# Alexyskoutnev/Quadruped-Trajectory-Optimization-Stack

Measured on AMD Instinct MI355X. Metric: NLP solves/sec (100-knot SOLO12 trot gait, 5 s horizon, converged to 1e-4); CoM L-inf vs TOWR in `parity`, higher is better.
Workload: dtype f64

## Files before the change

include/qtos_planner.h:

```cpp
#ifndef QTOS_PLANNER_H
#define QTOS_PLANNER_H

#ifdef __cplusplus
extern "C" {
#endif

#define QTOS_NEE 4
#define QTOS_MAX_PHASES 32
#define QTOS_START_DOUBLES 24
#define QTOS_CSV_COLS 37

typedef struct QtosParams {
  int n_phases[QTOS_NEE];
  double phase_dur[QTOS_NEE][QTOS_MAX_PHASES];
  double dt_base, dt_dyn, dt_rom;
  int force_polys_per_stance;
  double mass, gravity, inertia_b[9];
  double nominal_stance[QTOS_NEE][3], max_dev[3];
  double mu, f_max, t_swing_avg;
  int honor_start_velocity;
  int terrain_mode;
  int max_iter;
  double tol, mu_init, mu_min, delta_x, eps_dual;
  double slack_push;
// ... 100 lines not shown
  double step_size;
  double tol;
  double z_offset;
  double cell, origin_x, origin_y;
  double t_stop, stop_dist;
  int base;
  int clamp_x, advance_clock, hold_done;
  int n_paths, max_pieces;
  int n_maps, rows, cols;
} QtosPathGoal;
int qtos_path_goal_device(QtosPlanner *p, int B, const QtosPathGoal *g, const double *d_knots, const double *d_coef,
                          const int *d_n_pieces, const double *d_robot_goal , const int *d_path_id ,
                          const double *d_height_yx , const int *d_map_id , double *d_clock ,
                          const double *d_offset , const double *d_start , double *d_goal_out,
                          int *d_done , void *stream);
int qtos_path_goal(QtosPlanner *p, int B, const QtosPathGoal *g, const double *knots, const double *coef, const int *n_pieces,
                   const double *robot_goal, const int *path_id, const double *height_yx, const int *map_id, double *clock,
                   const double *offset, const double *start, double *goal_out, int *done);

typedef struct QtosPathPlan {
  int rows, cols;
  double cell, origin_x, origin_y;
  double height_bound;
  double step_size;
  int max_cells;
  int max_open;
  int max_pieces;
  int n_maps;
  int set_done;
} QtosPathPlan;
int qtos_path_plan_device(QtosPlanner *p, int B, const QtosPathPlan *g, const double *d_bool_maps, const int *d_map_id ,
                          const double *d_start, const double *d_robot_goal, double *d_knots, double *d_coef, int *d_n_pieces,
                          int *d_cells , int *d_n_cells, int *d_status, int *d_done , void *stream);
int qtos_path_plan(QtosPlanner *p, int B, const QtosPathPlan *g, const double *bool_maps, const int *map_id, const double *start,
                   const double *robot_goal, double *knots, double *coef, int *n_pieces, int *cells, int *n_cells, int *status, int *done);

typedef struct QtosProbe {
  int rows, cols;
  int n_maps;
  double cell;
  int scale;
  int multi_map_shift;
  double origin_shift;
  double z_offset;
  double nominal_stance[QTOS_NEE][3];
} QtosProbe;
int qtos_probe_device(QtosPlanner *p, const QtosProbe *g, const double *d_map_yx, int capacity, int *d_offsets, int *d_slot, int *d_patch,
                      double *d_start , double *d_goal , int *d_map_id , void *stream);
int qtos_probe(QtosPlanner *p, const QtosProbe *g, const double *map_yx, int capacity, int *offsets, int *slot, int *patch, double *start,
               double *goal, int *map_id);
int qtos_probe_stamp_device(QtosPlanner *p, const QtosProbe *g, const int *d_offsets, const int *d_slot, const int *d_patch ,
                            const int *d_status, double *d_bool_maps, void *stream);
int qtos_probe_stamp(QtosPlanner *p, const QtosProbe *g, const int *offsets, const int *slot, const int *patch, const int *status,
                     double *bool_maps);

#define QTOS_ENV_MAX_LEVELS 64
#define QTOS_ENV_MAX_DRAWS (1 << 24)
#define QTOS_ENV_LDS_BYTES 3568
typedef struct QtosTerrainEnv {
  int n_maps;
  int n_base;
  int rows, cols;
  int n_shift;
  int n_height;
  int climb;
  double delta;
} QtosTerrainEnv;
int qtos_terrain_env_device(QtosPlanner *p, const QtosTerrainEnv *g, const double *d_base_yx, const int *d_base_id ,
                            const unsigned long long *d_seed, int *d_draws , double *d_map_yx,
                            double *d_height_xy , int *d_status, void *stream);
int qtos_terrain_env(QtosPlanner *p, const QtosTerrainEnv *g, const double *base_yx, const int *base_id, const unsigned long long *seed,
                     int *draws, double *map_yx, double *height_xy, int *status);

int qtos_write_csv(const char *path, const double *rows, int n_rows, int n_threads);

int qtos_plan_submit(QtosPlanner *p, int B, const double *d_start, const double *d_goal,
                     const int *d_map_id, const double *d_warm, double *d_nodes_out,
                     int *d_status_out, int *d_iters_out, double *d_viol_out, void *stream);
int qtos_plan_poll(QtosPlanner *p, int *done);
int qtos_plan_wait(QtosPlanner *p);
int qtos_set_speculation(QtosPlanner *p, int max_blind_iterations);
int qtos_set_pattern_speculation(QtosPlanner *p, int on);
int qtos_env(const QtosPlanner *p, char *buf, int n);

int qtos_last_timing(QtosPlanner *p, double *kkt_seconds, int *kkt_launches, double *total_seconds,
                     int *iterations);
int qtos_last_timing_detail(QtosPlanner *p, double *out, int n_out);
int qtos_set_kernel_events(QtosPlanner *p, int on);
int qtos_set_report(QtosPlanner *p, int on);

#define QTOS_HIST_COLS 10
enum {
  QTOS_H_INF_PR = 0,
  QTOS_H_THETA,
  QTOS_H_MU,
  QTOS_H_DNORM,
  QTOS_H_ALPHA_PR,
  QTOS_H_ALPHA_DU,
  QTOS_H_LS,
  QTOS_H_KIND,
  QTOS_H_COMPL,
  QTOS_H_INF_DU
};

typedef struct QtosReport {
  int status;
  int iterations;
  int n_rows;
  int n_con_evals;
  int n_jac_evals;
  int n_factorizations;
  int n_chord_solves;
  int pad;
  double constraint_violation;
  double dual_infeasibility;
  double complementarity;
  double nlp_error;
} QtosReport;
int qtos_plan_report(QtosPlanner *p, int b, QtosReport *out, double *rows, int max_rows);
int qtos_analyze_counts(const QtosParams *params, long long *counts, int n);

int qtos_last_timing_chord(QtosPlanner *p, double *chord_seconds, int *chord_launches);
int qtos_plan_totals(QtosPlanner *p, long long *converged, long long *iterations, int reset);

int qtos_debug_eval(QtosPlanner *p, int B, const double *start, const double *goal,
                    const int *map_id, const double *nodes, double *g_out, double *J_out);
int qtos_debug_newton(QtosPlanner *p, int B, const double *start, const double *goal,
                      const int *map_id, const double *nodes, const double *sig, const double *w,
                      double *dx_out);
int qtos_debug_chord(QtosPlanner *p, int B, double *dx_out);
int qtos_project_nodes(QtosPlanner *p, int B, const double *nodes, double *nodes_out);
int qtos_debug_stream_len(const QtosPlanner *p);
int qtos_debug_read_stream(QtosPlanner *p, int b, double *out);
int qtos_debug_read_rhs(QtosPlanner *p, int b, double *out);
int qtos_debug_residual(QtosPlanner *p, int B, int refine, double *dx_out, double *res_rel_out);
int qtos_debug_structure(const QtosPlanner *p, int *row_kind, int *var_free, int *order);
int qtos_debug_factor(QtosPlanner *p, int b, double *panel_out, int *piv_slot_out);
int qtos_debug_initial_guess(QtosPlanner *p, int B, const double *start, const double *goal,
                             const int *map_id, double *nodes_out);
int qtos_debug_trace(QtosPlanner *p, int b, double *trace_out);
int qtos_debug_duals(QtosPlanner *p, int B, double *s, double *zl, double *zu, double *y);
int qtos_build_flags(void);
int qtos_kkt_kernel(const QtosPlanner *p, char *buf, int n);
int qtos_analyze_kernel(const QtosParams *params, char *buf, int n);

typedef struct QtosSelftest {
  int order_rule, front, n_stages;
  int n_problems;
  int worst_stage;
  int passed;
  double residual;
  double residual_refined;
  double max_factor;
  double growth_limit;
  double tol_residual;
  double seconds;
} QtosSelftest;
int qtos_planner_selftest(QtosPlanner *p, unsigned long long seed, double tol_residual, QtosSelftest *out);
int qtos_selftest_inputs(const QtosParams *params, unsigned long long seed, int b, double *dx0, double *sig, double *w);
unsigned long long qtos_selftest_bits(unsigned long long seed, int problem, int array, unsigned long long index);
int qtos_selftest_problem(const QtosParams *params, double *start, double *goal);
int qtos_planner_create_checked(const QtosParams *params, int max_batch, int device, int rules_mask, double tol_residual,
                                QtosPlanner **out, QtosSelftest *tried, int max_tried, int *n_tried);
int qtos_analyze_candidates(const QtosParams *params, int rules_mask, int *rules, int *fronts, int *stages, int n);

#ifdef __cplusplus
// ... 4 lines not shown
```

quadruped-trajectory-optimization-stack_amd/capi.py:

```python
import ctypes as C
import os

import numpy as np

_HERE = os.path.dirname(os.path.abspath(__file__))
LIB_PATH = os.path.join(_HERE, "csrc", os.environ.get("QTOS_LIB", "libqtos_planner.so"))
NEE, MAX_PHASES, START_DOUBLES, CSV_COLS = 4, 32, 24, 37


class QtosParams(C.Structure):
    _fields_ = [
        ("n_phases", C.c_int * NEE),
        ("phase_dur", (C.c_double * MAX_PHASES) * NEE),
        ("dt_base", C.c_double), ("dt_dyn", C.c_double), ("dt_rom", C.c_double),
        ("force_polys_per_stance", C.c_int),
        ("mass", C.c_double), ("gravity", C.c_double), ("inertia_b", C.c_double * 9),
        ("nominal_stance", (C.c_double * 3) * NEE), ("max_dev", C.c_double * 3),
        ("mu", C.c_double), ("f_max", C.c_double), ("t_swing_avg", C.c_double),
        ("honor_start_velocity", C.c_int), ("terrain_mode", C.c_int),
        ("max_iter", C.c_int),
        ("tol", C.c_double), ("mu_init", C.c_double), ("mu_min", C.c_double),
        ("delta_x", C.c_double), ("eps_dual", C.c_double), ("slack_push", C.c_double), ("warm_slack_push", C.c_double),
        ("stall_iters", C.c_int), ("hold_from", C.c_int), ("hold_weight", C.c_double), ("hold_tol", C.c_double),
        ("chord_tol", C.c_double),
# ... 154 lines not shown
    return g


class QtosProbe(C.Structure):
    _fields_ = [
        ("rows", C.c_int), ("cols", C.c_int), ("n_maps", C.c_int), ("cell", C.c_double), ("scale", C.c_int), ("multi_map_shift", C.c_int),
        ("origin_shift", C.c_double), ("z_offset", C.c_double), ("nominal_stance", (C.c_double * 3) * NEE),
    ]

    def copy(self):
        return QtosProbe.from_buffer_copy(self)


def probe_params(map_yx=None, multi_map_shift=1, scale=1, origin_shift=1.0, cell=0.1, z_offset=0.24,
                 nominal_stance=((0.21, 0.19, 0.0), (0.21, -0.19, 0.0), (-0.21, 0.19, 0.0), (-0.21, -0.19, 0.0))):
    g = QtosProbe()
    g.cell, g.scale, g.multi_map_shift = float(cell), int(scale), int(multi_map_shift)
    g.origin_shift, g.z_offset = float(origin_shift), float(z_offset)
    for e in range(NEE):
        for k in range(3):
            g.nominal_stance[e][k] = float(nominal_stance[e][k])
    if map_yx is not None:
        is_shape = isinstance(map_yx, (tuple, list)) and len(map_yx) in (2, 3) and all(isinstance(v, (int, np.integer)) for v in map_yx)
        shape = tuple(int(v) for v in (map_yx if is_shape else np.shape(map_yx)))
        if len(shape) not in (2, 3):
            raise ValueError("map_yx is n_maps x rows x cols or rows x cols, or that shape")
        g.n_maps, g.rows, g.cols = (1,) + shape if len(shape) == 2 else shape
    return g


class QtosTerrainEnv(C.Structure):
    _fields_ = [
        ("n_maps", C.c_int), ("n_base", C.c_int), ("rows", C.c_int), ("cols", C.c_int), ("n_shift", C.c_int), ("n_height", C.c_int),
        ("climb", C.c_int), ("delta", C.c_double),
    ]

    def copy(self):
        return QtosTerrainEnv.from_buffer_copy(self)


ENV_MAX_LEVELS, ENV_MAX_DRAWS, ENV_LDS_BYTES = 64, 1 << 24, 3568


def terrain_env_params(base_yx=None, n_maps=None, n_shift=10, n_height=10, climb=False, delta=0.005):
    g = QtosTerrainEnv()
    g.n_shift, g.n_height, g.climb, g.delta = int(n_shift), int(n_height), int(bool(climb)), float(delta)
    if base_yx is not None:
        is_shape = isinstance(base_yx, (tuple, list)) and len(base_yx) in (2, 3) and all(isinstance(v, (int, np.integer)) for v in base_yx)
        shape = tuple(int(v) for v in (base_yx if is_shape else np.shape(base_yx)))
        if len(shape) not in (2, 3):
            raise ValueError("base_yx is n_base x rows x cols or rows x cols, or that shape")
        g.n_base, g.rows, g.cols = (1,) + shape if len(shape) == 2 else shape
        g.n_maps = g.n_base
    if n_maps is not None:
        g.n_maps = int(n_maps)
    return g


class SelftestError(RuntimeError):

    def __init__(self, attempts):
        self.attempts = attempts
        RuntimeError.__init__(self, "no elimination order passed the KKT self-test: " + "; ".join(a.describe() for a in attempts))


MAX_TRIED = 3

EXPORTS = [
    "qtos_planner_create", "qtos_planner_destroy", "qtos_planner_dims", "qtos_last_error",
    "qtos_set_heightfields", "qtos_plan_batch", "qtos_plan_batch_device", "qtos_sample_csv",
    "qtos_sample_csv_device", "qtos_last_timing", "qtos_debug_eval", "qtos_debug_newton",
    "qtos_debug_structure", "qtos_debug_trace", "qtos_debug_factor", "qtos_analyze", "qtos_analyze_sweep", "qtos_analyze_kron",
    "qtos_set_init_table", "qtos_debug_initial_guess", "qtos_shift_warm", "qtos_shift_warm_device",
    "qtos_last_timing_chord", "qtos_debug_chord", "qtos_plan_totals",
    "qtos_plan_submit", "qtos_plan_poll", "qtos_plan_wait", "qtos_set_speculation", "qtos_debug_residual", "qtos_project_nodes",
    "qtos_debug_stream_len", "qtos_debug_read_stream", "qtos_debug_read_rhs", "qtos_build_flags", "qtos_kkt_kernel",
    "qtos_last_timing_detail", "qtos_set_pattern_speculation", "qtos_env", "qtos_analyze_two_ended", "qtos_analyze_order", "qtos_set_kernel_events",
    "qtos_write_csv", "qtos_set_report", "qtos_plan_report", "qtos_analyze_counts", "qtos_debug_duals", "qtos_analyze_kernel",
    "qtos_planner_selftest", "qtos_planner_create_checked", "qtos_analyze_candidates", "qtos_selftest_inputs", "qtos_selftest_bits",
    "qtos_selftest_problem", "qtos_handover", "qtos_handover_device", "qtos_stitch", "qtos_stitch_device",
    "qtos_path_goal", "qtos_path_goal_device", "qtos_path_plan", "qtos_path_plan_device",
    "qtos_probe", "qtos_probe_device", "qtos_probe_stamp", "qtos_probe_stamp_device",
    "qtos_terrain_env", "qtos_terrain_env_device", "qtos_set_heightfields_device",
]

_lib = None


def load():
    global _lib
    if _lib is not None:
        return _lib
    if not os.path.exists(LIB_PATH):
        raise OSError("HIP planner library not built: %s (run __graft_entry__.build()); "
                      "this package has no CPU fallback" % LIB_PATH)
    try:
        import importlib.util
        spec = importlib.util.find_spec("torch")
        for loc in (spec.submodule_search_locations or []) if spec else []:
            hip = os.path.join(loc, "lib", "libamdhip64.so")
            if os.path.exists(hip):
                C.CDLL(hip, mode=C.RTLD_GLOBAL)
                break
    except Exception:
        pass
    lib = C.CDLL(LIB_PATH)
    _warn_if_two_hip_runtimes()
    dp, ip, vp = C.POINTER(C.c_double), C.POINTER(C.c_int), C.c_void_p
    lib.qtos_planner_create.argtypes = [C.POINTER(QtosParams), C.c_int, C.c_int, C.POINTER(vp)]
    lib.qtos_planner_destroy.argtypes = [vp]
    lib.qtos_planner_destroy.restype = None
    lib.qtos_planner_dims.argtypes = [vp, C.POINTER(QtosDims)]
    lib.qtos_last_error.argtypes = [vp]
    lib.qtos_last_error.restype = C.c_char_p
    lib.qtos_set_heightfields.argtypes = [vp, C.c_int, dp, C.c_int, C.c_int, C.c_double, C.c_double, C.c_double]
    lib.qtos_plan_batch.argtypes = [vp, C.c_int, dp, dp, ip, dp, dp, ip, ip, dp]
    lib.qtos_plan_batch_device.argtypes = [vp, C.c_int, vp, vp, vp, vp, vp, vp, vp, vp, vp]
    lib.qtos_sample_csv.argtypes = [vp, C.c_int, dp, dp, C.c_double, C.c_int, dp]
    lib.qtos_write_csv.argtypes = [C.c_char_p, dp, C.c_int, C.c_int]
    lib.qtos_sample_csv_device.argtypes = [vp, C.c_int, vp, vp, C.c_double, C.c_int, vp, vp]
    lib.qtos_last_timing.argtypes = [vp, dp, ip, dp, ip]
    lib.qtos_debug_eval.argtypes = [vp, C.c_int, dp, dp, ip, dp, dp, dp]
    lib.qtos_debug_newton.argtypes = [vp, C.c_int, dp, dp, ip, dp, dp, dp, dp]
    lib.qtos_debug_structure.argtypes = [vp, ip, ip, ip]
    lib.qtos_debug_trace.argtypes = [vp, C.c_int, dp]
    lib.qtos_debug_factor.argtypes = [vp, C.c_int, dp, ip]
    lib.qtos_analyze.argtypes = [C.POINTER(QtosParams), C.POINTER(QtosDims), ip, C.c_int]
    lib.qtos_analyze_sweep.argtypes = [C.POINTER(QtosParams), ip, ip, ip, ip, ip, C.c_int]
    lib.qtos_analyze_kron.argtypes = [C.POINTER(QtosParams), ip, ip, ip, dp]
    lib.qtos_set_init_table.argtypes = [vp, C.c_int, dp, C.c_int, dp, dp]
    lib.qtos_debug_initial_guess.argtypes = [vp, C.c_int, dp, dp, ip, dp]
    if hasattr(lib, "qtos_last_timing_chord"):
        lib.qtos_last_timing_chord.argtypes = [vp, dp, ip]
    if hasattr(lib, "qtos_plan_totals"):
        lib.qtos_plan_totals.argtypes = [vp, C.POINTER(C.c_longlong), C.POINTER(C.c_longlong), C.c_int]
        lib.qtos_debug_chord.argtypes = [vp, C.c_int, dp]
    if hasattr(lib, "qtos_project_nodes"):
        lib.qtos_project_nodes.argtypes = [vp, C.c_int, dp, dp]
    if hasattr(lib, "qtos_debug_residual"):
        lib.qtos_debug_residual.argtypes = [vp, C.c_int, C.c_int, dp, dp]
    if hasattr(lib, "qtos_plan_submit"):
        lib.qtos_plan_submit.argtypes = [vp, C.c_int, vp, vp, vp, vp, vp, vp, vp, vp, vp]
        lib.qtos_plan_poll.argtypes = [vp, ip]
        lib.qtos_plan_wait.argtypes = [vp]
        lib.qtos_set_speculation.argtypes = [vp, C.c_int]
    if hasattr(lib, "qtos_last_timing_detail"):
        lib.qtos_last_timing_detail.argtypes = [vp, dp, C.c_int]
        lib.qtos_set_pattern_speculation.argtypes = [vp, C.c_int]
        if hasattr(lib, "qtos_set_kernel_events"):
            lib.qtos_set_kernel_events.argtypes = [vp, C.c_int]
        lib.qtos_env.argtypes = [vp, C.c_char_p, C.c_int]
    if hasattr(lib, "qtos_analyze_two_ended"):
        lib.qtos_analyze_two_ended.argtypes = [C.POINTER(QtosParams), ip, C.c_int]
    if hasattr(lib, "qtos_analyze_order"):
        lib.qtos_analyze_order.argtypes = [C.POINTER(QtosParams), ip, C.c_int]
    if hasattr(lib, "qtos_shift_warm"):
        lib.qtos_shift_warm.argtypes = [vp, C.c_int, dp, dp, dp, dp, ip, dp]
        lib.qtos_shift_warm_device.argtypes = [vp, C.c_int, vp, vp, vp, vp, vp, vp, vp]
    if hasattr(lib, "qtos_set_report"):
        lib.qtos_set_report.argtypes = [vp, C.c_int]
        lib.qtos_plan_report.argtypes = [vp, C.c_int, C.POINTER(QtosReport), dp, C.c_int]
        lib.qtos_debug_duals.argtypes = [vp, C.c_int, dp, dp, dp, dp]
    if hasattr(lib, "qtos_analyze_counts"):
        lib.qtos_analyze_counts.argtypes = [C.POINTER(QtosParams), C.POINTER(C.c_longlong), C.c_int]
    if hasattr(lib, "qtos_analyze_kernel"):
        lib.qtos_analyze_kernel.argtypes = [C.POINTER(QtosParams), C.c_char_p, C.c_int]
    if hasattr(lib, "qtos_planner_selftest"):
        ull = C.c_ulonglong
        lib.qtos_planner_selftest.argtypes = [vp, ull, C.c_double, C.POINTER(QtosSelftest)]
        lib.qtos_planner_create_checked.argtypes = [C.POINTER(QtosParams), C.c_int, C.c_int, C.c_int, C.c_double, C.POINTER(vp),
                                                    C.POINTER(QtosSelftest), C.c_int, ip]
        lib.qtos_analyze_candidates.argtypes = [C.POINTER(QtosParams), C.c_int, ip, ip, ip, C.c_int]
        lib.qtos_selftest_inputs.argtypes = [C.POINTER(QtosParams), ull, C.c_int, dp, dp, dp]
        lib.qtos_selftest_bits.argtypes = [ull, C.c_int, C.c_int, ull]
        lib.qtos_selftest_bits.restype = ull
        lib.qtos_selftest_problem.argtypes = [C.POINTER(QtosParams), dp, dp]
    if hasattr(lib, "qtos_handover"):
        lib.qtos_handover.argtypes = [vp, C.c_int, C.POINTER(QtosHandover), dp, dp, dp, dp, dp, ip]
        lib.qtos_handover_device.argtypes = [vp, C.c_int, C.POINTER(QtosHandover), vp, vp, vp, vp, vp, vp, vp]
    if hasattr(lib, "qtos_stitch"):
        llp = C.POINTER(C.c_longlong)
        lib.qtos_stitch.argtypes = [vp, C.c_int, C.POINTER(QtosStitch), dp, ip, dp, dp, llp]
        lib.qtos_stitch_device.argtypes = [vp, C.c_int, C.POINTER(QtosStitch), vp, vp, vp, vp, vp, vp]
    if hasattr(lib, "qtos_path_goal"):
        lib.qtos_path_goal.argtypes = [vp, C.c_int, C.POINTER(QtosPathGoal), dp, dp, ip, dp, ip, dp, ip, dp, dp, dp, dp, ip]
        lib.qtos_path_goal_device.argtypes = [vp, C.c_int, C.POINTER(QtosPathGoal)] + [vp] * 13
    if hasattr(lib, "qtos_path_plan"):
        lib.qtos_path_plan.argtypes = [vp, C.c_int, C.POINTER(QtosPathPlan), dp, ip, dp, dp, dp, dp, ip, ip, ip, ip, ip]
        lib.qtos_path_plan_device.argtypes = [vp, C.c_int, C.POINTER(QtosPathPlan)] + [vp] * 12
    if hasattr(lib, "qtos_probe"):
        lib.qtos_probe.argtypes = [vp, C.POINTER(QtosProbe), dp, C.c_int, ip, ip, ip, dp, dp, ip]
        lib.qtos_probe_device.argtypes = [vp, C.POINTER(QtosProbe), vp, C.c_int] + [vp] * 7
        lib.qtos_probe_stamp.argtypes = [vp, C.POINTER(QtosProbe), ip, ip, ip, ip, dp]
        lib.qtos_probe_stamp_device.argtypes = [vp, C.POINTER(QtosProbe)] + [vp] * 6
    if hasattr(lib, "qtos_terrain_env"):
        u64p = C.POINTER(C.c_uint64)
        lib.qtos_terrain_env.argtypes = [vp, C.POINTER(QtosTerrainEnv), dp, ip, u64p, ip, dp, dp, ip]
        lib.qtos_terrain_env_device.argtypes = [vp, C.POINTER(QtosTerrainEnv)] + [vp] * 8
    if hasattr(lib, "qtos_set_heightfields_device"):
        lib.qtos_set_heightfields_device.argtypes = [vp, C.c_int, vp, C.c_int, C.c_int, C.c_double, C.c_double, C.c_double, vp]
    _lib = lib
    return lib


def _warn_if_two_hip_runtimes():
    try:
        paths = {ln.split()[-1] for ln in open("/proc/self/maps") if "libamdhip64" in ln}
        real = {os.path.realpath(q) for q in paths}
        if len(real) > 1:
            import warnings
            warnings.warn("two HIP runtimes are mapped into this process (%s): the planner library and PyTorch do not share "
                          "one libamdhip64; GPU work may fail or see no device" % ", ".join(sorted(real)))
    except OSError:
        pass


def _dp(a):
    return None if a is None else a.ctypes.data_as(C.POINTER(C.c_double))


def _ip(a):
    return None if a is None else a.ctypes.data_as(C.POINTER(C.c_int))


def params_from_config(cfg):
    p = QtosParams()
    for e in range(NEE):
        d = cfg.phase_durations[e]
        if len(d) > MAX_PHASES:
            raise ValueError("at most %d phases per foot" % MAX_PHASES)
        p.n_phases[e] = len(d)
        for k, v in enumerate(d):
            p.phase_dur[e][k] = float(v)
        for k in range(3):
            p.nominal_stance[e][k] = float(cfg.nominal_stance[e][k])
    p.dt_base, p.dt_dyn, p.dt_rom = cfg.dt_base, cfg.dt_dynamic, cfg.dt_range_of_motion
    p.force_polys_per_stance = cfg.force_polys_per_stance
    p.mass, p.gravity = cfg.mass, cfg.gravity
    for k, v in enumerate(np.asarray(cfg.inertia_b, float).reshape(9)):
        p.inertia_b[k] = v
    for k in range(3):
        p.max_dev[k] = cfg.max_deviation[k]
    p.mu, p.f_max, p.t_swing_avg = cfg.friction, cfg.force_limit, cfg.t_swing_avg
    p.honor_start_velocity = int(cfg.honor_start_velocity)
    p.terrain_mode = int(cfg.terrain_mode)
    p.max_iter, p.tol = cfg.max_iter, cfg.tol
    p.mu_init, p.mu_min, p.delta_x, p.eps_dual = cfg.mu_init, cfg.mu_min, cfg.delta_x, cfg.eps_dual
    p.slack_push = cfg.slack_push
    p.warm_slack_push = cfg.warm_slack_push
    p.stall_iters = cfg.stall_iters
    p.hold_from, p.hold_weight, p.hold_tol = cfg.foothold_hold_from, cfg.foothold_hold_weight, cfg.foothold_hold_tol
    p.chord_tol = cfg.chord_tol
    p.reduce_base = int(cfg.reduce_base)
    p.chord_max, p.chord_shrink = int(cfg.chord_max), float(cfg.chord_shrink)
    p.stall_alpha = float(cfg.stall_alpha)
    p.reduce_swing = int(getattr(cfg, "reduce_swing", False))
    p.mu_superlinear = int(getattr(cfg, "mu_superlinear", False))
    return p


def build_flags():
    return int(load().qtos_build_flags())


def analyze(cfg):
    lib = load()
    p = params_from_config(cfg)
    d = QtosDims()
    act = np.zeros(4096, np.int32)
    rc = lib.qtos_analyze(C.byref(p), C.byref(d), _ip(act), act.size)
    if rc != 0:
        raise ValueError("qtos_analyze failed (%d)" % rc)
    return d, act[:d.n_stages].copy()


def analyze_counts(cfg):
    lib = load()
    if not hasattr(lib, "qtos_analyze_counts"):
        return None
    p = params_from_config(cfg)
    c = (C.c_longlong * 2)()
    if lib.qtos_analyze_counts(C.byref(p), c, 2) != 2:
        raise ValueError("qtos_analyze_counts failed")
    return int(c[0]), int(c[1])


def analyze_kernel(cfg):
    lib = load()
    p = params_from_config(cfg)
    buf = C.create_string_buffer(64)
    n = lib.qtos_analyze_kernel(C.byref(p), buf, 64)
    if n < 0:
        raise ValueError("qtos_analyze_kernel failed (%d)" % n)
    return buf.value.decode()


def _selftest_lib():
    lib = load()
    if not hasattr(lib, "qtos_planner_selftest"):
        raise RuntimeError("this build of the planner library has no KKT self-test (qtos_planner_selftest)")
    return lib


def analyze_candidates(cfg, rules_mask=0):
    lib = _selftest_lib()
    p = params_from_config(cfg)
    a = [np.zeros(MAX_TRIED, np.int32) for _ in range(3)]
    n = lib.qtos_analyze_candidates(C.byref(p), int(rules_mask), _ip(a[0]), _ip(a[1]), _ip(a[2]), MAX_TRIED)
    if n < 0:
        raise ValueError("qtos_analyze_candidates failed (%d)" % n)
    return [(int(a[0][i]), int(a[1][i]), int(a[2][i])) for i in range(min(n, MAX_TRIED))]


def selftest_inputs(cfg, seed, b):
    lib = _selftest_lib()
    p = params_from_config(cfg)
    d, _ = analyze(cfg)
    dx0, sig, w = np.zeros(d.n_vars), np.zeros(d.n_cons), np.zeros(d.n_cons)
    rc = lib.qtos_selftest_inputs(C.byref(p), int(seed), int(b), _dp(dx0), _dp(sig), _dp(w))
    if rc != 0:
        raise ValueError("qtos_selftest_inputs failed (%d)" % rc)
    return dx0, sig, w


def selftest_bits(seed, problem, array, index):
    return int(_selftest_lib().qtos_selftest_bits(int(seed), int(problem), int(array), int(index)))


def selftest_problem(cfg):
    lib = _selftest_lib()
    p = params_from_config(cfg)
    start, goal = np.zeros(START_DOUBLES), np.zeros(3)
    if lib.qtos_selftest_problem(C.byref(p), _dp(start), _dp(goal)) != 0:
        raise ValueError("qtos_selftest_problem failed")
    return start, goal


def analyze_order(cfg):
    lib = load()
    p = params_from_config(cfg)
    a = np.full(1 << 15, -2, np.int32)
    n = lib.qtos_analyze_order(C.byref(p), _ip(a), a.size)
    if n < 0 or n > a.size:
        raise ValueError("qtos_analyze_order failed (%d)" % n)
    return a[:n].copy()


def analyze_two_ended(cfg):
    lib = load()
    p = params_from_config(cfg)
    a = np.zeros(20, np.int32)
    rc = lib.qtos_analyze_two_ended(C.byref(p), _ip(a), a.size)
    if rc != 0:
        raise ValueError("qtos_analyze_two_ended failed (%d)" % rc)
    keys = ("stages_now", "front_now", "split_stage", "stages_left", "stages_right", "sep_unknowns", "stages_sep", "front_left", "front_right",
            "front_sep", "serial_steps", "peak_left", "peak_right", "lds_now", "lds_panels", "lds_records", "lds_cells", "lds_two_chains_as_is",
            "lds_two_chains_lean", "lds_limit")
    return {k: int(v) for k, v in zip(keys, a)}


def analyze_kron(cfg):
    lib = load()
    p = params_from_config(cfg)
    a = [np.zeros(1, np.int32) for _ in range(3)]
    w = np.zeros(1)
    rc = lib.qtos_analyze_kron(C.byref(p), _ip(a[0]), _ip(a[1]), _ip(a[2]), _dp(w))
    if rc != 0:
        raise ValueError("qtos_analyze_kron failed (%d)" % rc)
    return int(a[0][0]), int(a[1][0]), int(a[2][0]), float(w[0])
# ... 295 lines not shown
        g.n_maps, (g.rows, g.cols) = len(offsets) - 1, tuple(shape)[-2:]
        slot = np.ascontiguousarray(slot, np.int32)
        patch = None if patch is None else np.ascontiguousarray(patch, np.int32).reshape(-1, 3)
        status = np.ascontiguousarray(status, np.int32).reshape(-1)
        N = int(offsets[-1])
        if slot.size != g.n_maps * g.rows * max(g.cols // 2 - 1, 0) or len(status) < N or (patch is not None and len(patch) < N):
            raise ValueError("slot is n_maps x rows x (cols // 2 - 1); patch (or None) and status hold offsets[-1] entries")
        out = np.zeros((g.n_maps, g.rows, g.cols))
        self._chk(self.lib.qtos_probe_stamp(self.h, C.byref(g), _ip(offsets), _ip(slot), _ip(patch), _ip(status), _dp(out)), "probe_stamp")
        return out

    def has_terrain_env(self):
        return hasattr(self.lib, "qtos_terrain_env")

    def terrain_env(self, base_yx, seed, draws=None, base_id=None, params=None, map_yx=None, height_xy=None):
        if not self.has_terrain_env():
            raise RuntimeError("this build of the planner library has no terrain-env kernel (qtos_terrain_env)")
        base = np.ascontiguousarray(base_yx, np.float64)
        base = base[None] if base.ndim == 2 else base
        seed = np.ascontiguousarray([int(v) for v in np.ravel(seed)], np.uint64)
        g = (params or terrain_env_params()).copy()
        g.n_maps, (g.n_base, g.rows, g.cols) = len(seed), base.shape
        draws = np.zeros(g.n_maps, np.int32) if draws is None else np.array(draws, np.int32).reshape(g.n_maps)
        bid = None if base_id is None else np.ascontiguousarray(base_id, np.int32).reshape(g.n_maps)
        out_m = np.zeros((g.n_maps, g.rows, g.cols)) if map_yx is None else map_yx
        out_h = np.zeros((g.n_maps, g.cols, g.rows)) if height_xy is None else height_xy
        for a in (out_m, out_h):
            if a.dtype != np.float64 or not a.flags.c_contiguous or a.size != g.n_maps * g.rows * g.cols:
                raise ValueError("map_yx and height_xy are contiguous float64 arrays of n_maps x rows x cols values")
        status = np.zeros(g.n_maps, np.int32)
        self._chk(self.lib.qtos_terrain_env(self.h, C.byref(g), _dp(base), _ip(bid), seed.ctypes.data_as(C.POINTER(C.c_uint64)), _ip(draws),
                                            _dp(out_m), _dp(out_h), _ip(status)), "terrain_env")
        return dict(map_yx=out_m, height_xy=out_h, draws=draws, status=status)

    def set_heightfields_device(self, height_xy, cell, x0=-1.0, y0=-1.0, stream=None):
        import torch
        if not hasattr(self.lib, "qtos_set_heightfields_device"):
            raise RuntimeError("this build of the planner library has no qtos_set_heightfields_device")
        t = height_xy[None] if height_xy.dim() == 2 else height_xy
        if not t.is_cuda or t.device.index != self.device or t.dtype != torch.float64 or t.dim() != 3:
            raise ValueError("height_xy is a float64 tensor n_maps x nx x ny on the planner's device")
        stream = torch.cuda.current_stream(t.device) if stream is None else stream
        with torch.cuda.stream(stream):
            t = t.contiguous()
            self._chk(self.lib.qtos_set_heightfields_device(self.h, t.shape[0], t.data_ptr(), t.shape[1], t.shape[2], cell, x0, y0,
                                                            C.c_void_p(stream.cuda_stream)), "set_heightfields_device")

    def set_init_table(self, dx=None, dy=None, nodes=None):
        if dx is None:
            self._chk(self.lib.qtos_set_init_table(self.h, 0, None, 0, None, None), "set_init_table")
            self.init_table = None
            return
        dx = np.ascontiguousarray(dx, np.float64)
        dy = np.ascontiguousarray(dy, np.float64)
        nodes = np.ascontiguousarray(nodes, np.float64).reshape(len(dy), len(dx), self.n)
        self._chk(self.lib.qtos_set_init_table(self.h, len(dx), _dp(dx), len(dy), _dp(dy), _dp(nodes)), "set_init_table")
        self.init_table = (dx, dy, nodes)

    def build_init_table(self, dx=None, dy=None, z=0.24):
        from . import workloads
        T = self.dims.duration
        dx = np.asarray(dx if dx is not None else np.linspace(0.03, 0.15, 5) * T, np.float64)
        dy = np.asarray(dy if dy is not None else [-0.1, 0.0, 0.1], np.float64)
        self.set_init_table()
        start = np.repeat(workloads.rest_start(0.0, 0.0, z)[None], len(dx) * len(dy), 0)
        goal = np.array([[x, y, z] for y in dy for x in dx])
        nodes = np.empty((len(goal), self.n))
        for i in range(0, len(goal), self.max_batch):
            sl = slice(i, i + self.max_batch)
            nodes[sl], status, _, _ = self.plan(start[sl], goal[sl])
            if (status != 0).any():
                raise RuntimeError("a nominal plan of the table did not converge")
        self.set_init_table(dx, dy, nodes)
        return dx, dy

    def initial_guess(self, start, goal, map_id=None):
        start = np.ascontiguousarray(start, np.float64).reshape(-1, START_DOUBLES)
        goal = np.ascontiguousarray(goal, np.float64).reshape(-1, 3)
        out = np.empty((start.shape[0], self.n))
        mid = None if map_id is None else np.ascontiguousarray(map_id, np.int32)
        self._chk(self.lib.qtos_debug_initial_guess(self.h, start.shape[0], _dp(start), _dp(goal), _ip(mid), _dp(out)), "initial_guess")
        return out

    def kkt_kernel(self):
        buf = C.create_string_buffer(64)
        self.lib.qtos_kkt_kernel.argtypes = [C.c_void_p, C.c_char_p, C.c_int]
        self._chk(min(self.lib.qtos_kkt_kernel(self.h, buf, 64), 0), "kkt_kernel")
        return buf.value.decode()

    def timing(self):
        k, t = C.c_double(), C.c_double()
        nl, it = C.c_int(), C.c_int()
        self._chk(self.lib.qtos_last_timing(self.h, C.byref(k), C.byref(nl), C.byref(t), C.byref(it)), "last_timing")
        out = dict(kkt_seconds=k.value, kkt_launches=nl.value, total_seconds=t.value, iterations=it.value)
        if hasattr(self.lib, "qtos_last_timing_chord"):
            c, nc = C.c_double(), C.c_int()
            self._chk(self.lib.qtos_last_timing_chord(self.h, C.byref(c), C.byref(nc)), "last_timing_chord")
            out.update(chord_seconds=c.value, chord_launches=nc.value)
        return out

    def totals(self, reset=False):
        c, n = C.c_longlong(), C.c_longlong()
        self._chk(self.lib.qtos_plan_totals(self.h, C.byref(c), C.byref(n), int(bool(reset))), "plan_totals")
        return c.value, n.value

    def debug_eval(self, start, goal, nodes, map_id=None, jac=True):
        start = np.ascontiguousarray(start, np.float64).reshape(-1, START_DOUBLES)
        goal = np.ascontiguousarray(goal, np.float64).reshape(-1, 3)
        nodes = np.ascontiguousarray(nodes, np.float64).reshape(-1, self.n)
        B = start.shape[0]
        g = np.empty((B, self.m))
        J = np.empty((B, self.m, self.n)) if jac else None
        mid = None if map_id is None else np.ascontiguousarray(map_id, np.int32)
        self._chk(self.lib.qtos_debug_eval(self.h, B, _dp(start), _dp(goal), _ip(mid), _dp(nodes), _dp(g), _dp(J)), "debug_eval")
        return g, J

    def debug_newton(self, start, goal, nodes, sig, w, map_id=None):
        start = np.ascontiguousarray(start, np.float64).reshape(-1, START_DOUBLES)
        goal = np.ascontiguousarray(goal, np.float64).reshape(-1, 3)
        nodes = np.ascontiguousarray(nodes, np.float64).reshape(-1, self.n)
        B = start.shape[0]
        sig = np.ascontiguousarray(sig, np.float64).reshape(B, self.m)
        w = np.ascontiguousarray(w, np.float64).reshape(B, self.m)
        dx = np.empty((B, self.n))
        mid = None if map_id is None else np.ascontiguousarray(map_id, np.int32)
        self._chk(self.lib.qtos_debug_newton(self.h, B, _dp(start), _dp(goal), _ip(mid), _dp(nodes), _dp(sig), _dp(w), _dp(dx)), "debug_newton")
        return dx

    def debug_chord(self, B):
        dx = np.empty((B, self.n))
        self._chk(self.lib.qtos_debug_chord(self.h, B, _dp(dx)), "debug_chord")
        return dx

    def project(self, nodes):
        nodes = np.ascontiguousarray(nodes, np.float64).reshape(-1, self.n)
        out = np.empty_like(nodes)
        self._chk(self.lib.qtos_project_nodes(self.h, nodes.shape[0], _dp(nodes), _dp(out)), "project_nodes")
        return out

    def debug_residual(self, B, refine=False):
        dx = np.empty((B, self.n))
        res = np.empty(B)
        self._chk(self.lib.qtos_debug_residual(self.h, B, int(bool(refine)), _dp(dx), _dp(res)), "debug_residual")
        return dx, res

    def structure(self):
        rk = np.empty(self.m, np.int32)
        vf = np.empty(self.n, np.int32)
        order = np.empty(self.dims.n_stages * self.dims.pivots, np.int32)
        self.lib.qtos_debug_structure(self.h, _ip(rk), _ip(vf), _ip(order))
        return rk, vf, order

    def factor(self, b):
        d = self.dims
        pan = np.zeros((d.n_stages, d.front + 1, 16))
        ps = np.zeros((d.n_stages, 16), dtype=np.int32)
        self._chk(self.lib.qtos_debug_factor(self.h, b, _dp(pan), _ip(ps)), "qtos_debug_factor")
        cols = np.array([4 * (c & 3) + (c >> 2) for c in range(16)])
        pan[:, 1:, :] = pan[:, 1:, :][:, :, cols]
        return pan, ps

    def trace(self, b):
        t = np.zeros((self.cfg.max_iter + 1, 4))
        rows = self.lib.qtos_debug_trace(self.h, b, _dp(t))
        return t[:max(rows, 0)]
```

quadruped-trajectory-optimization-stack_amd/csrc/env.hpp:

```cpp
#pragma once
#include <algorithm>
#include <cstdio>
#include <cstdlib>
#include <string>

namespace qtos {

struct QtosEnv {
  int kkt = 0;
  int lanes = 1;
  int short_stages = -1;
  int sweep_ds = 1;
  int spec_jac = 1;
  int spec_pattern = 1;
  int kron = 0;
  int order = -1;
  int place = 0;
  int debug = 0;
  int debug_kron = 0;
  std::string dump_first;

  static QtosEnv parse() {
    QtosEnv e;
    auto num = [](const char *name, int dflt) { const char *v = getenv(name); return v ? atoi(v) : dflt; };
    e.kkt = num("QTOS_KKT", 0);
    e.lanes = std::max(1, std::min(4, num("QTOS_LANES", 1)));
    if (getenv("QTOS_SHORT_STAGES")) e.short_stages = num("QTOS_SHORT_STAGES", 1) != 0;
    if (num("QTOS_NO_SHORT_STAGES", 0) != 0) e.short_stages = 0;
    e.sweep_ds = num("QTOS_SWEEP_DS", 1) != 0;
    e.spec_jac = num("QTOS_SPEC_JAC", 1) != 0;
    e.spec_pattern = num("QTOS_SPEC_PATTERN", 1) != 0;
    e.kron = num("QTOS_KRON", 0) != 0;
    e.place = num("QTOS_PLACE", 0);
    if (getenv("QTOS_ORDER")) e.order = std::max(0, std::min(2, num("QTOS_ORDER", 0)));
    e.debug = getenv("QTOS_DEBUG_SYMBOLIC2") ? 2 : (getenv("QTOS_DEBUG_SYMBOLIC") ? 1 : 0);
    e.debug_kron = getenv("QTOS_DEBUG_KRON") != nullptr;
    if (const char *v = getenv("QTOS_DUMP_FIRST")) e.dump_first = v;
    return e;
  }
  std::string describe() const {
    char b[320];
    snprintf(b, sizeof(b), "QTOS_KKT=%d QTOS_LANES=%d QTOS_SHORT_STAGES=%s QTOS_SWEEP_DS=%d QTOS_SPEC_JAC=%d QTOS_SPEC_PATTERN=%d QTOS_KRON=%d QTOS_PLACE=%d QTOS_ORDER=%s QTOS_DEBUG_SYMBOLIC=%d",
             kkt, lanes, short_stages < 0 ? "unset" : (short_stages ? "1" : "0"), sweep_ds, spec_jac, spec_pattern, kron, place,
             order < 0 ? "unset" : (order == 2 ? "2" : order ? "1" : "0"), debug);
    return b;
  }
};

}
```

quadruped-trajectory-optimization-stack_amd/csrc/kernels.hpp:

```cpp
#pragma once
#include <hip/hip_runtime.h>

#include "model.hpp"
#include "symbolic.hpp"

namespace qtos {

typedef double d4_t __attribute__((ext_vector_type(4)));
typedef double d2_t __attribute__((ext_vector_type(2)));
typedef int i4_t __attribute__((ext_vector_type(4)));

struct TerrDev {
  int vx, vy, vz, row;
  int px, py, pz;
  int d0, d1;
  int pad;
  double ex, ey;
};

struct DevPlan {
  int n_vars, n_cons, n_stages, front;
  int n_sol, n_rec;
  const int *rec_var, *rec_col;
  const double *rec_w;
  int n_coef, n_pz;
  int n_psw;
  const int *psw_var, *psw_src;
  const double *psw_w;
  const int *pc_var, *pz_var, *pz_col;
  const double *pc_w, *pz_w;
  int n_dyn, n_rom, n_terr, n_force, n_lin, n_blocks;
  const DynInst *dyn;
  const RomInst *rom;
  const i4_t *pre_dyn_var, *pre_rom_var;
  const d2_t *pre_dyn_wa, *pre_dyn_wb, *pre_rom_wa, *pre_rom_wb;
  const TerrDev *terr;
  const ForceInst *force;
  const LinRow *lin;
  const PackedTerm1 *dyn_t1, *rom_t1;
  const PackedTerm3 *dyn_t3;
  const double *lin_coef;
  int n_lin_coef, coef_in_lds;
  const int *dyn_t1_off, *dyn_t3_off;
  int n_rom_t1;
  int rom_chunk;
  const int *rom_t1_off;
  int dyn_chunk;
  const double *table, *tab_dx, *tab_dy;
  int tab_ndx, tab_ndy;
  int off_lin, off_ang, off_eem[NEE];
  const int *cont;
  int n_cont;
  int spec_jac;
  int hold_from;
  double hold_weight, hold_tol;
  const unsigned *amask;
  const unsigned *amask2;
  const int *nxt_pack;
  const unsigned short *ctab;
  int n_cells;
  double chord_tol, chord_shrink;
  int chord_max;
  int n_unknowns;
  const int *rhs_ptr, *rhs_gpos, *rhs_row;
  int n_rhs_ent, rhs_chunk;
  const int *kx_ptr, *kx_col, *kx_pos;
  const int *rtab;
  const Block *blocks;
  const int *block_cols;
  const IqRow *iq_rows;
  int n_iq_rows;
  const SwTask *sw_tasks;
  const int *sw_cpos, *sw_c16;
  int sw_steps, sw_on;
  const int *iq_idx, *eq_idx;
  const double *iq_lo, *iq_hi;
  int n_iq, n_eqw;
  const double *g_static;
  const int *piv_slot, *piv_unknown;
  const double *piv_diag;
  const StageDesc *stages;
  const EqEntry *eq_entries;
  const EqRhs *eq_rhs;
  const IqBlock *iq_blocks;
  const short *iq_slots;
  int max_stage_g;
  const int *srec, *srec_off, *pack_src, *drec_off;
  const int *diag_pos;
  const unsigned *pair_groups;
  const int *eq_pos, *rhs_pos, *sig_pos, *w_pos;
  int max_srec, max_drec, stream_len;
  const double *con_lo, *con_hi;
  const int *row_kind;
  const InitDesc *init;
  const double *var_time;
  double mass, gravity, Ib[9], mu_fric, f_max, T;
  double nominal[NEE][3];
  double tol, mu_init, mu_min, delta_x, eps_dual, slack_push, warm_slack_push;
  int mu_superlinear;
  int max_iter, stall_iters;
  double stall_alpha;
  const double *height;
  int n_maps, hnx, hny, terrain_mode;
  double hcell, hx0, hy0;
  long long g_doubles, panel_stride;
  int kron_lds_off;
};

struct DevWork {
  const double *start, *goal, *warm;
  const int *map_id;
  double *x, *g, *gt, *s, *zl, *zu, *ds, *dzl, *dzu, *sig, *w, *G, *panel, *dx, *stream;
  double *mu, *viol, *trace;
  double *best_viol, *xbest;
  int *held;
  int *best_it;
  int *status, *iters, *done, *n_active;
  int *chord;
  int *chord_run;
  int *jam;
  double *rhs;
  double *minv;
  double *sol;
  double *sol0, *dx0, *ur;
  double *nodes_out, *viol_out;
  int *status_out, *iters_out;
  unsigned long long *totals;
// ... 158 lines not shown
  bool cx = false, cy = false;
  if (fx <= 0) { fx = 0; cx = true; }
  if (fx >= mx) { fx = mx; cx = true; }
  if (fy <= 0) { fy = 0; cy = true; }
  if (fy >= my) { fy = my; cy = true; }
  int ix = (int)floor(fx), iy = (int)floor(fy);
  ix = min(ix, P.hnx - 2); iy = min(iy, P.hny - 2);
  ix = max(ix, 0); iy = max(iy, 0);
  const double u = fx - ix, v = fy - iy;
  const int ix1 = P.hnx > 1 ? ix + 1 : ix, iy1 = P.hny > 1 ? iy + 1 : iy;
  const double h00 = H[ix * P.hny + iy], h10 = H[ix1 * P.hny + iy], h01 = H[ix * P.hny + iy1],
               h11 = H[ix1 * P.hny + iy1];
  t.h = h00 * (1 - u) * (1 - v) + h10 * u * (1 - v) + h01 * (1 - u) * v + h11 * u * v;
  const double c = P.hcell;
  t.hx = cx ? 0 : ((h10 - h00) * (1 - v) + (h11 - h01) * v) / c;
  t.hy = cy ? 0 : ((h01 - h00) * (1 - u) + (h11 - h10) * u) / c;
  t.hxy = (cx || cy) ? 0 : (h11 - h10 - h01 + h00) / (c * c);
  return t;
}
__device__ inline void terrain_basis(const Terr &t, int which, double b[3], double bx[3], double by[3]) {
  double v[3], vx[3] = {0, 0, 0}, vy[3] = {0, 0, 0};
  if (which == 0) { v[0] = -t.hx; v[1] = -t.hy; v[2] = 1; vx[1] = -t.hxy; vy[0] = -t.hxy; }
  else if (which == 1) { v[0] = 1; v[1] = 0; v[2] = t.hx; vy[2] = t.hxy; }
  else { v[0] = 0; v[1] = 1; v[2] = t.hy; vx[2] = t.hxy; }
  const double nn = sqrt(v[0] * v[0] + v[1] * v[1] + v[2] * v[2]);
  for (int i = 0; i < 3; ++i) b[i] = v[i] / nn;
  const double px = b[0] * vx[0] + b[1] * vx[1] + b[2] * vx[2];
  const double py = b[0] * vy[0] + b[1] * vy[1] + b[2] * vy[2];
  for (int i = 0; i < 3; ++i) { bx[i] = (vx[i] - b[i] * px) / nn; by[i] = (vy[i] - b[i] * py) / nn; }
}


template <bool JAC>
__device__ inline void eval_dyn(const DevPlan &P, const DynInst &I, const double *vin, double *g, double *loc,
                                const double th[3], const double thd[3], const double thdd[3], const Trig &tg) {
  const double r[3] = {vin[0], vin[1], vin[2]}, a[3] = {vin[3], vin[4], vin[5]};
  double ga[3], gl[3];
  dyn_angular<double>(P.Ib, th, thd, thdd, tg, ga);
  gl[0] = P.mass * a[0]; gl[1] = P.mass * a[1]; gl[2] = P.mass * a[2] + P.mass * P.gravity;
  const bool jac = JAC && I.in_kkt;
  double sf[3] = {0, 0, 0};
#pragma unroll
  for (int e = 0; e < NEE; ++e) {
    const double *pe = vin + 15 + 3 * e, *f = vin + 27 + 3 * e;
    const double d[3] = {r[0] - pe[0], r[1] - pe[1], r[2] - pe[2]};
    ga[0] -= f[1] * d[2] - f[2] * d[1];
    ga[1] -= f[2] * d[0] - f[0] * d[2];
    ga[2] -= f[0] * d[1] - f[1] * d[0];
    gl[0] -= f[0]; gl[1] -= f[1]; gl[2] -= f[2];
    if (jac) {
#pragma unroll
      for (int i = 0; i < 3; ++i) { sf[i] += f[i]; loc[30 + 3 * e + i] = f[i]; loc[42 + 3 * e + i] = d[i]; }
    }
  }
  if (jac) { loc[27] = sf[0]; loc[28] = sf[1]; loc[29] = sf[2]; }
#pragma unroll
  for (int i = 0; i < 3; ++i) { g[I.row0 + i] = ga[i]; g[I.row0 + 3 + i] = gl[i]; }
}
template <int WHAT>
__device__ inline void eval_dyn_pass(const DevPlan &P, const DynInst &I, double *loc, const double th[3],
                                     const double thd[3], const double thdd[3], const Trig &tg) {
  if (!I.in_kkt) return;
#pragma unroll
  for (int j = 0; j < 3; ++j) {
    D1 t0[3], t1[3], t2[3], o[3];
#pragma unroll
    for (int i = 0; i < 3; ++i) {
      t0[i] = {th[i], (WHAT == 0 && i == j) ? 1.0 : 0.0};
      t1[i] = {thd[i], (WHAT == 1 && i == j) ? 1.0 : 0.0};
      t2[i] = {thdd[i], (WHAT == 2 && i == j) ? 1.0 : 0.0};
    }
    dyn_angular<D1>(P.Ib, t0, t1, t2, tg, o);
#pragma unroll
    for (int i = 0; i < 3; ++i) loc[9 * WHAT + 3 * i + j] = o[i].d;
  }
}

#ifndef TERM1_UNROLL
#define TERM1_UNROLL 24
#endif
#ifndef TERM3_UNROLL
#define TERM3_UNROLL 8
#endif
__device__ inline void write_terms1(const PackedTerm1 *T, int i0, int i1, const double *loc, const double *coef, double *G) {
  const int nt = blockDim.x;
  constexpr int UN = TERM1_UNROLL;
  for (int i = i0 + threadIdx.x; i < i1; i += UN * nt) {
    PackedTerm1 t[UN];
#pragma unroll
    for (int u = 0; u < UN; ++u) t[u] = T[min(i + u * nt, i1 - 1)];
#pragma unroll
    for (int u = 0; u < UN; ++u)
      if (i + u * nt < i1) G[t[u].pos] = coef[t[u].ai] * loc[t[u].off];
  }
}
__device__ inline void write_terms3(const PackedTerm3 *T, int i0, int i1, const double *loc, const double *coef, double *G) {
  const int nt = blockDim.x;
  constexpr int UN = TERM3_UNROLL;
  for (int i = i0 + threadIdx.x; i < i1; i += UN * nt) {
    PackedTerm3 t[UN];
#pragma unroll
    for (int u = 0; u < UN; ++u) t[u] = T[min(i + u * nt, i1 - 1)];
#pragma unroll
    for (int u = 0; u < UN; ++u)
      if (i + u * nt < i1)
        G[t[u].pos] = loc[t[u].off[0]] * coef[t[u].ai[0]] + loc[t[u].off[1]] * coef[t[u].ai[1]] + loc[t[u].off[2]] * coef[t[u].ai[2]];
  }
}

template <bool JAC>
__device__ inline void eval_rom(const DevPlan &P, const RomInst &I, const double *vin, double *g, double *loc) {
  const double *r = vin, *th = vin + 3, *pe = vin + 6;
  const double d[3] = {pe[0] - r[0], pe[1] - r[1], pe[2] - r[2]};
  double R[9];
  const Trig tg = trig_of(th);
  rotation<double>(th, tg, R);
#pragma unroll
  for (int i = 0; i < 3; ++i) g[I.row0 + i] = R[i] * d[0] + R[3 + i] * d[1] + R[6 + i] * d[2];
  if (JAC) {
#pragma unroll
    for (int i = 0; i < 9; ++i) loc[i] = R[i];
#pragma unroll
    for (int j = 0; j < 3; ++j) {
      D1 t0[3];
#pragma unroll
      for (int i = 0; i < 3; ++i) t0[i] = {th[i], i == j ? 1.0 : 0.0};
      D1 Rd[9];
      rotation<D1>(t0, tg, Rd);
#pragma unroll
      for (int i = 0; i < 3; ++i) loc[9 + 3 * i + j] = Rd[i].d * d[0] + Rd[3 + i].d * d[1] + Rd[6 + i].d * d[2];
    }
  }
}

template <bool JAC>
__device__ inline void eval_terr(const DevPlan &P, const TerrDev &I, int map, const double *x, double *g, double *Gp, int hold = -1) {
  const Terr t = terrain_at(P, map, x[I.vx], x[I.vy]);
  g[I.row] = x[I.vz] - t.h;
  if (JAC) {
    const double wgt = hold > 0 ? P.hold_weight : P.delta_x;
    if (I.d0 >= 0) Gp[I.d0] = wgt + I.ex;
    if (I.d1 >= 0) Gp[I.d1] = wgt + I.ey;
    if (I.px >= 0) Gp[I.px] = -t.hx;
    if (I.py >= 0) Gp[I.py] = -t.hy;
    if (I.pz >= 0) Gp[I.pz] = 1.0;
  }
}

template <bool JAC>
__device__ inline void eval_force(const DevPlan &P, const ForceInst &I, int map, const double *x, double *g, double *Gp) {
  const double f[3] = {x[I.vf[0]], x[I.vf[1]], x[I.vf[2]]};
  const Terr t = terrain_at(P, map, x[I.vsx], x[I.vsy]);
  double b[3][3], bx[3][3], by[3][3];
  for (int w = 0; w < 3; ++w) terrain_basis(t, w, b[w], bx[w], by[w]);
  const double mu = P.mu_fric;
  const double ct[5][3] = {{1, 0, 0}, {-mu, 1, 0}, {mu, 1, 0}, {-mu, 0, 1}, {mu, 0, 1}};
  const int nc = I.ncol;
  double *G = JAC ? Gp + I.goff : nullptr;
  for (int row = 0; row < 5; ++row) {
    double v[3], vx[3], vy[3];
    for (int i = 0; i < 3; ++i) {
      v[i] = ct[row][0] * b[0][i] + ct[row][1] * b[1][i] + ct[row][2] * b[2][i];
      vx[i] = ct[row][0] * bx[0][i] + ct[row][1] * bx[1][i] + ct[row][2] * bx[2][i];
      vy[i] = ct[row][0] * by[0][i] + ct[row][1] * by[1][i] + ct[row][2] * by[2][i];
    }
    g[I.row0 + row] = f[0] * v[0] + f[1] * v[1] + f[2] * v[2];
    if (JAC) {
      for (int i = 0; i < 3; ++i)
        if (I.cf[i] >= 0) G[row * nc + I.cf[i]] = v[i];
      if (I.csx >= 0) G[row * nc + I.csx] = f[0] * vx[0] + f[1] * vx[1] + f[2] * vx[2];
      if (I.csy >= 0) G[row * nc + I.csy] = f[0] * vy[0] + f[1] * vy[1] + f[2] * vy[2];
    }
  }
}

__device__ __forceinline__ int eval_loc_offset(int n_vars) { return (n_vars + 1) & ~1; }
constexpr int DYN_VIN = 39, ROM_VIN = 9;
__device__ __forceinline__ int fresh(int v) {
  asm volatile("" : "+v"(v));
  return v;
}
__device__ __forceinline__ void wg_lds_barrier() { asm volatile("s_waitcnt lgkmcnt(0)\n\ts_barrier" ::: "memory"); }
#ifndef QTOS_EVAL_LDSBAR
#define QTOS_EVAL_LDSBAR 1
#endif
#if QTOS_EVAL_LDSBAR
#define EVAL_BARRIER() wg_lds_barrier()
#else
#define EVAL_BARRIER() __syncthreads()
#endif
template <bool JAC>
__device__ inline void eval_all(const DevPlan &P, int map, const double *xg, double *g, double *G, double *lds, double *dbg = nullptr,
                                int hold = -1) {
  const int tid = threadIdx.x, nt = blockDim.x;
#ifdef QTOS_STAMPS
  unsigned long long et0 = 0; int ei = 0;
#define ESTAMP() do { __syncthreads(); if (tid == 0 && dbg) { unsigned long long t_; asm volatile("s_memtime %0\n\ts_waitcnt lgkmcnt(0)" : "=s"(t_) :: "memory"); dbg[ei++] = (double)(t_ - et0); et0 = t_; } } while (0)
  if (tid == 0) asm volatile("s_memtime %0\n\ts_waitcnt lgkmcnt(0)" : "=s"(et0) :: "memory");
#else
#define ESTAMP() do {} while (0)
#endif
  double *x = lds, *loc = lds + eval_loc_offset(P.n_vars);
  double *vin = loc + max(DYN_LOC * P.dyn_chunk, ROM_LOC * P.rom_chunk);
  double *coef_lds = vin + max(DYN_VIN * P.dyn_chunk, ROM_VIN * P.rom_chunk);
  const double *coef = P.coef_in_lds ? coef_lds : P.lin_coef;
  if (xg)
    for (int v = fresh(tid); v < P.n_vars; v += nt) x[v] = xg[v];
  if (JAC && P.coef_in_lds)
    for (int v = fresh(tid); v < P.n_lin_coef; v += nt) coef_lds[v] = P.lin_coef[v];
  EVAL_BARRIER();
  for (int c0 = 0, ch = 0; c0 < P.n_dyn; c0 += P.dyn_chunk, ++ch) {
    const int cnt = min(P.dyn_chunk, P.n_dyn - c0);
    if (c0) EVAL_BARRIER();
    vec_prepass(P.pre_dyn_var + c0 * DYN_VIN, P.pre_dyn_wa + c0 * DYN_VIN, P.pre_dyn_wb + c0 * DYN_VIN, cnt * DYN_VIN, x, vin);
    EVAL_BARRIER();
    ESTAMP();
    if (JAC) {
      const int cpad = (cnt + 63) & ~63;
      for (int it = tid; it < 4 * cpad; it += nt) {
        const int what = it / cpad, i = it - what * cpad;
        if (i >= cnt) continue;
        double *li = loc + (size_t)i * DYN_LOC;
        const DynInst &I = P.dyn[c0 + i];
        const double *vi = vin + (size_t)i * DYN_VIN, *th = vi + 6, *thd = vi + 9, *thdd = vi + 12;
        const Trig tg = trig_of(th);
        if (what == 0) eval_dyn<true>(P, I, vi, g, li, th, thd, thdd, tg);
        else if (what == 1) eval_dyn_pass<0>(P, I, li, th, thd, thdd, tg);
        else if (what == 2) eval_dyn_pass<1>(P, I, li, th, thd, thdd, tg);
        else eval_dyn_pass<2>(P, I, li, th, thd, thdd, tg);
      }
      EVAL_BARRIER();
      ESTAMP();
      write_terms1(P.dyn_t1, P.dyn_t1_off[ch], P.dyn_t1_off[ch + 1], loc, coef, G);
      write_terms3(P.dyn_t3, P.dyn_t3_off[ch], P.dyn_t3_off[ch + 1], loc, coef, G);
      EVAL_BARRIER();
      ESTAMP();
    } else {
      for (int i = tid; i < cnt; i += nt) {
        const DynInst &I = P.dyn[c0 + i];
        const double *vi = vin + (size_t)i * DYN_VIN, *th = vi + 6, *thd = vi + 9, *thdd = vi + 12;
        eval_dyn<false>(P, I, vi, g, nullptr, th, thd, thdd, trig_of(th));
      }
      ESTAMP();
    }
  }
  for (int c0 = 0, ch = 0; c0 < P.n_rom; c0 += P.rom_chunk, ++ch) {
    const int cnt = min(P.rom_chunk, P.n_rom - c0);
    EVAL_BARRIER();
    vec_prepass(P.pre_rom_var + c0 * ROM_VIN, P.pre_rom_wa + c0 * ROM_VIN, P.pre_rom_wb + c0 * ROM_VIN, cnt * ROM_VIN, x, vin);
    EVAL_BARRIER();
    for (int i = tid; i < cnt; i += nt) eval_rom<JAC>(P, P.rom[c0 + i], vin + (size_t)i * ROM_VIN, g, JAC ? loc + (size_t)i * ROM_LOC : nullptr);
    if (!JAC) ESTAMP();
    if (JAC) {
      EVAL_BARRIER();
      ESTAMP();
      write_terms1(P.rom_t1, P.rom_t1_off[ch], P.rom_t1_off[ch + 1], loc, coef, G);
      ESTAMP();
    }
  }
  {
    const int rt = nt - 1 - tid;
    for (int base = 0; base < max(max(P.n_force + P.n_terr, 1), (P.n_lin + 1) / 2); base += nt) {
      const int fi = base + rt, ti = base + rt - P.n_force, l0 = 2 * (base + tid), l1 = l0 + 1;
      const bool hf = fi < P.n_force, ht = ti >= 0 && ti < P.n_terr, h0 = l0 < P.n_lin, h1 = l1 < P.n_lin;
      ForceInst FI;
      TerrDev TI;
      LinRow L0, L1;
      if (hf) FI = P.force[fi];
      if (ht) TI = P.terr[ti];
      if (h0) L0 = P.lin[l0];
      if (h1) L1 = P.lin[l1];
      if (hf) eval_force<JAC>(P, FI, map, x, g, G);
      if (ht) eval_terr<JAC>(P, TI, map, x, g, G, hold);
      auto lin_row = [&](const LinRow &L) __attribute__((always_inline)) {
        double xv[8], acc = 0;
#pragma unroll
        for (int k = 0; k < 8; ++k) xv[k] = x[k < L.n ? L.var[k] : 0];
#pragma unroll
        for (int k = 0; k < 8; ++k)
          if (k < L.n) acc += L.coef[k] * xv[k];
        g[L.row] = acc;
      };
      if (h0) lin_row(L0);
      if (h1) lin_row(L1);
    }
  }
  ESTAMP();
}

#ifndef QTOS_ET
#define QTOS_ET 512
#endif
constexpr int ET = QTOS_ET;
template <int OP>
__device__ __forceinline__ double wg_op(double a, double b) { return OP == 0 ? a + b : (OP == 1 ? fmax(a, b) : fmin(a, b)); }
template <int CTRL>
__device__ __forceinline__ double wg_dpp(double v) {
  return __hiloint2double(__builtin_amdgcn_update_dpp(0, __double2hiint(v), CTRL, 0xf, 0xf, false),
                          __builtin_amdgcn_update_dpp(0, __double2loint(v), CTRL, 0xf, 0xf, false));
}
template <int OP, int NT = ET>
__device__ inline double wg_reduce(double v, double *scratch) {
  static_assert(NT % 64 == 0 && (NT / 64 & (NT / 64 - 1)) == 0, "wg_reduce: a power-of-two number of full waves");
  constexpr int NW = NT / 64;
#ifdef QTOS_CHECKS
  if (blockDim.x != NT) __builtin_trap();
#endif
  const int tid = threadIdx.x, lane = tid & 63;
  wg_lds_barrier();
  scratch[tid] = v;
  wg_lds_barrier();
  double a[NW];
#pragma unroll
  for (int w = 0; w < NW; ++w) a[w] = scratch[64 * w + lane];
#pragma unroll
  for (int s = NW / 2; s > 0; s >>= 1)
#pragma unroll
    for (int w = 0; w < s; ++w) a[w] = wg_op<OP>(a[w], a[w + s]);
  double r = a[0];
  {
    int lo = __double2loint(r), hi = __double2hiint(r);
    auto l = __builtin_amdgcn_permlane32_swap(lo, lo, false, false);
    auto h = __builtin_amdgcn_permlane32_swap(hi, hi, false, false);
    r = wg_op<OP>(__hiloint2double(h[0], l[0]), __hiloint2double(h[1], l[1]));
    lo = __double2loint(r); hi = __double2hiint(r);
    auto l2 = __builtin_amdgcn_permlane16_swap(lo, lo, false, false);
    auto h2 = __builtin_amdgcn_permlane16_swap(hi, hi, false, false);
    r = wg_op<OP>(__hiloint2double(h2[0], l2[0]), __hiloint2double(h2[1], l2[1]));
  }
  r = wg_op<OP>(r, wg_dpp<0x128>(r));
  r = wg_op<OP>(r, wg_dpp<0x12C>(r));
  r = wg_op<OP>(r, wg_dpp<0x12E>(r));
  r = wg_op<OP>(r, wg_dpp<0x12F>(r));
  return __hiloint2double(__builtin_amdgcn_readfirstlane(__double2hiint(r)), __builtin_amdgcn_readfirstlane(__double2loint(r)));
}

__device__ inline void barrier_terms(const DevPlan &P, const double *__restrict__ g, const double *__restrict__ s,
                                     const double *__restrict__ zl, const double *__restrict__ zu, double mu,
                                     double *__restrict__ sig, double *__restrict__ w, double *__restrict__ stream) {
#pragma unroll 4
  for (int i = threadIdx.x; i < P.n_eqw; i += blockDim.x) {
    const int r = P.eq_idx[i];
    stream[P.rhs_pos[r]] = -g[r];
  }
#pragma unroll 4
  for (int i = threadIdx.x; i < P.n_iq; i += blockDim.x) {
    const int r = P.iq_idx[i];
    const double l = P.iq_lo[i], u = P.iq_hi[i];
    const bool hl = l > -1e19, hu = u < 1e19;
    const double dl = hl ? s[r] - l : 1.0, du = hu ? u - s[r] : 1.0;
    const double zql = zl[r] / dl, zqu = zu[r] / du, ml = mu / dl, mq = mu / du;
    const double sg = (hl ? zql : 0.0) + (hu ? zqu : 0.0);
    const double gmu = -(hl ? ml : 0.0) + (hu ? mq : 0.0);
    const double wr = sg * (g[r] - s[r]) + gmu;
    sig[r] = sg;
    w[r] = wr;
    stream[P.sig_pos[r]] = sg;
    stream[P.w_pos[r]] = wr;
  }
}

__device__ inline void infeasibility(const DevPlan &P, const double *__restrict__ g, const double *__restrict__ s,
                                     double *scratch, double &viol, double &theta) {
  double v = 0, t = 0;
#pragma unroll 4
  for (int i = threadIdx.x; i < P.n_eqw; i += blockDim.x) {
    const double gr = g[P.eq_idx[i]];
    if (!(gr == gr)) { v = t = INFINITY; continue; }
    v = fmax(v, fabs(gr));
    t = fmax(t, fabs(gr));
// ... 604 lines not shown
  double rds[KR];
#pragma unroll
  for (int k = 0; k < KR; ++k) {
    const int ic = ic_row(k);
    rl[k] = P.iq_lo[ic]; ru[k] = P.iq_hi[ic];
    rs[k] = s[rr[k]]; rzl[k] = zl[rr[k]]; rzu[k] = zu[rr[k]]; rg[k] = g[rr[k]]; rds[k] = ds[rr[k]];
  }
#pragma unroll
  for (int k = 0; k < KE; ++k) eg[k] = g[er[k]];
  auto dz_row = [&](bool valid, double l, double u, double sv, double d, double zlv, double zuv, bool &hl, bool &hu, double &dl, double &du,
                    double &a_, double &c_) __attribute__((always_inline)) {
    hl = valid && l > -1e19; hu = valid && u < 1e19;
    dl = hl ? sv - l : 1.0; du = hu ? u - sv : 1.0;
    const double ml = mu / dl, zql = zlv / dl, mq = mu / du, zqu = zuv / du;
    a_ = ml - zlv - zql * d; c_ = mq - zuv + zqu * d;
  };
  auto ratio_row = [&](bool valid, double l, double u, double sv, double d, double zlv, double zuv, double &a, double &c) __attribute__((always_inline)) {
    bool hl, hu;
    double dl, du, a_, c_;
    dz_row(valid, l, u, sv, d, zlv, zuv, hl, hu, dl, du, a_, c_);
    a = hl ? a_ : 0.0;
    c = hu ? c_ : 0.0;
    const double r1 = tau * dl / -d, r2 = tau * du / d, r3 = tau * zlv / -a_, r4 = tau * zuv / -c_;
    amax = (hl && d < 0) ? fmin(amax, r1) : amax;
    amax = (hu && d > 0) ? fmin(amax, r2) : amax;
    az = (hl && a_ < 0) ? fmin(az, r3) : az;
    az = (hu && c_ < 0) ? fmin(az, r4) : az;
  };
#pragma unroll
  for (int k = 0; k < KR; ++k) {
    double a, c;
    ratio_row(tid + k * nt < P.n_iq, rl[k], ru[k], rs[k], rds[k], rzl[k], rzu[k], a, c);
  }
  for (int i = tid + KR * nt; i < P.n_iq; i += nt) {
    const int r = P.iq_idx[i];
    double a, c;
    ratio_row(true, P.iq_lo[i], P.iq_hi[i], s[r], ds[r], zl[r], zu[r], a, c);
    dzl[r] = a;
    dzu[r] = c;
  }
  amax = wg_reduce<2>(amax, scratch);
  az = wg_reduce<2>(az, scratch);
  auto l1_rows = [&](const double (&gI)[KR], const double (&gE)[KE], const double (&sI)[KR], const double (&dI)[KR], const double *__restrict__ gm,
                     double alq) __attribute__((always_inline)) {
    double t = 0;
#pragma unroll
    for (int k = 0; k < KE; ++k)
      if (tid + k * nt < P.n_eqw) t += fabs(gE[k]);
    for (int i = fresh(tid) + KE * nt; i < P.n_eqw; i += nt) t += fabs(gm[P.eq_idx[i]]);
#pragma unroll
    for (int k = 0; k < KR; ++k)
      if (tid + k * nt < P.n_iq) t += fabs(gI[k] - (sI[k] + alq * dI[k]));
    for (int i = fresh(tid) + KR * nt; i < P.n_iq; i += nt) {
      const int r = P.iq_idx[i];
      t += fabs(gm[r] - (s[r] + alq * ds[r]));
    }
    return wg_reduce<0>(t, scratch);
  };
  const double th0 = l1_rows(rg, eg, rs, rds, g, 0.0);
  KSTAMP(1);
  double al = amax, th = 0;
  double rgt[KR], egt[KE];
  bool lin_done = false;
  int n_trials = 0;
  for (int ls = 0; ls < 6; ++ls) {
    ++n_trials;
    for (int v = tid; v < n; v += blockDim.x) evl[v] = x[v] + al * dx[v];
    __syncthreads();
    double *gv = (spec && ls == 0) ? g : gt;
    if (spec && ls == 0)
      eval_all<true>(P, map, nullptr, g, W.stream + (size_t)b * P.stream_len, evl, (W.trace && it == 1) ? W.trace + ((size_t)b * (P.max_iter + 1) + 72) * 4 : nullptr, held0);
    else
      eval_all<false>(P, map, nullptr, gt, nullptr, evl, (W.trace && it == 1 && ls == 0) ? W.trace + ((size_t)b * (P.max_iter + 1) + 76) * 4 : nullptr);
    __syncthreads();
    double st_[KR], dst[KR];
    int rk[KR], ek[KE];
    fresh_rows(rr, rk);
    fresh_rows(er, ek);
#pragma unroll
    for (int k = 0; k < KR; ++k) { rgt[k] = gv[rk[k]]; st_[k] = s[rk[k]]; dst[k] = ds[rk[k]]; }
#pragma unroll
    for (int k = 0; k < KE; ++k) egt[k] = gv[ek[k]];
    th = l1_rows(rgt, egt, st_, dst, gv, al);
    if (th <= (1.0 - 1e-4 * al) * th0 || th < 1e-9) { lin_done = spec && ls == 0; break; }
    if (ls < 5) al *= 0.5;
  }
  KSTAMP(2);
  const bool reject = was_chord && al != 1.0;
  if (reject) {
    al = 0.0; az = 0.0; th = 0.0;
    int rk[KR], ek[KE];
    fresh_rows(rr, rk);
    fresh_rows(er, ek);
#pragma unroll
    for (int k = 0; k < KR; ++k) rg[k] = g[rk[k]];
#pragma unroll
    for (int k = 0; k < KE; ++k) eg[k] = g[ek[k]];
  } else {
    for (int v = tid; v < n; v += blockDim.x) x[v] = evl[v];
#pragma unroll
    for (int k = 0; k < KR; ++k) rg[k] = rgt[k];
#pragma unroll
    for (int k = 0; k < KE; ++k) eg[k] = egt[k];
    if (!rows_in_regs && !lin_done) {
#pragma unroll 4
      for (int r = tid; r < m; r += blockDim.x) g[r] = gt[r];
    }
  }
  auto update_row = [&](double l, double u, double &sv, double d, double &zlv, double &zuv, double dl_, double du_) __attribute__((always_inline)) {
    const bool hl = l > -1e19, hu = u < 1e19;
    const double sn = sv + al * d;
    sv = sn;
    const double a = zlv + az * dl_, c = zuv + az * du_;
    const double kap = 1e10;
    const double gl = hl ? sn - l : 1.0, gu = hu ? u - sn : 1.0;
    const double lo_l = mu / (kap * gl), hi_l = kap * mu / gl, lo_u = mu / (kap * gu), hi_u = kap * mu / gu;
    zlv = hl ? fmin(fmax(a, lo_l), hi_l) : a;
    zuv = hu ? fmin(fmax(c, lo_u), hi_u) : c;
  };
  int rk[KR];
  fresh_rows(rr, rk);
#pragma unroll
  for (int k = 0; k < KR; ++k) {
    const int ic = ic_row(k);
    rl[k] = P.iq_lo[ic]; ru[k] = P.iq_hi[ic];
    rs[k] = s[rk[k]]; rzl[k] = zl[rk[k]]; rzu[k] = zu[rk[k]]; rds[k] = ds[rk[k]];
  }
#pragma unroll
  for (int k = 0; k < KR; ++k) {
    const bool valid = tid + k * nt < P.n_iq;
    double rdzl, rdzu;
    {
      bool hl, hu;
      double dl, du, a_, c_;
      dz_row(valid, rl[k], ru[k], rs[k], rds[k], rzl[k], rzu[k], hl, hu, dl, du, a_, c_);
      rdzl = hl ? a_ : 0.0;
      rdzu = hu ? c_ : 0.0;
    }
    double sv = rs[k], zlv = rzl[k], zuv = rzu[k];
    update_row(rl[k], ru[k], sv, rds[k], zlv, zuv, rdzl, rdzu);
    if (valid) {
      rs[k] = sv; rzl[k] = zlv; rzu[k] = zuv;
      s[rk[k]] = sv; zl[rk[k]] = zlv; zu[rk[k]] = zuv;
    }
  }
  for (int i = fresh(tid) + KR * nt; i < P.n_iq; i += nt) {
    const int r = P.iq_idx[i];
    double sv = s[r], zlv = zl[r], zuv = zu[r];
    update_row(P.iq_lo[i], P.iq_hi[i], sv, ds[r], zlv, zuv, dzl[r], dzu[r]);
    s[r] = sv; zl[r] = zlv; zu[r] = zuv;
  }
  if (al > 0.3) mu = P.mu_superlinear ? fmax(fmax(P.mu_min, P.tol), fmin(0.2 * mu, mu * sqrt(mu))) : fmax(P.mu_min, 0.2 * mu);
  __syncthreads();
  double viol, theta;
  {
    double v = 0, t = 0;
    auto eq_row = [&](double gr) __attribute__((always_inline)) {
      if (!(gr == gr)) { v = t = INFINITY; return; }
      v = fmax(v, fabs(gr));
      t = fmax(t, fabs(gr));
    };
    auto iq_row = [&](double gr, double sr, double l, double u) __attribute__((always_inline)) {
      if (!(gr == gr) || !(sr == sr)) { v = t = INFINITY; return; }
      v = fmax(v, fmax(l - gr, gr - u));
      t = fmax(t, fabs(gr - sr));
    };
#pragma unroll
    for (int k = 0; k < KE; ++k)
      if (tid + k * nt < P.n_eqw) eq_row(eg[k]);
    for (int i = fresh(tid) + KE * nt; i < P.n_eqw; i += nt) eq_row(g[P.eq_idx[i]]);
#pragma unroll
    for (int k = 0; k < KR; ++k)
      if (tid + k * nt < P.n_iq) iq_row(rg[k], rs[k], rl[k], ru[k]);
    for (int i = fresh(tid) + KR * nt; i < P.n_iq; i += nt) {
      const int r = P.iq_idx[i];
      iq_row(g[r], s[r], P.iq_lo[i], P.iq_hi[i]);
    }
    viol = wg_reduce<1>(v, scratch);
    theta = wg_reduce<1>(t, scratch);
  }
  KSTAMP(3);
  double h_dn = 0.0, h_cp = 0.0;
  if (W.hist) {
    double d = 0.0, c = 0.0;
    for (int v = tid; v < n; v += nt) { const double a = fabs(dx[v]); d = a == a ? fmax(d, a) : INFINITY; }
#pragma unroll
    for (int k = 0; k < KR; ++k)
      if (tid + k * nt < P.n_iq) c = fmax(c, compl_row(rl[k], ru[k], rs[k], rzl[k], rzu[k]));
    for (int i = fresh(tid) + KR * nt; i < P.n_iq; i += nt) { const int r = P.iq_idx[i]; c = fmax(c, compl_row(P.iq_lo[i], P.iq_hi[i], s[r], zl[r], zu[r])); }
    h_dn = wg_reduce<1>(d, scratch);
    h_cp = wg_reduce<1>(c, scratch);
  }
  const bool conv = viol <= P.tol && theta <= P.tol;
  const bool bad = !(viol < INFINITY) || !(th < INFINITY);
  const bool improved = !conv && !bad && viol < best_viol;
  const int jam = (P.stall_alpha > 0 && !reject && al < P.stall_alpha) ? jam_prev + 1 : 0;
  const bool stalled = !conv && !bad && ((!improved && P.stall_iters > 0 && it + 1 - best_it >= P.stall_iters) || jam >= 2);
  if (improved)
    for (int v = tid; v < n; v += blockDim.x) W.xbest[(size_t)b * n + v] = x[v];
  const bool restore = stalled || (bad && best_viol < INFINITY);
  if (restore)
    for (int v = tid; v < n; v += blockDim.x) x[v] = W.xbest[(size_t)b * n + v];
  if (tid == 0) {
    W.mu[b] = mu;
    W.viol[b] = restore ? (improved ? viol : best_viol) : viol;
    W.iters[b] = it + 1;
    W.jam[b] = jam;
    if (improved) { W.best_viol[b] = viol; W.best_it[b] = it + 1; }
    record_trace(P, W, b, it + 1, viol, theta, al, mu);
    if (W.hist) {
      double *h = W.hist + ((size_t)b * (P.max_iter + 1) + it + 1) * HIST_COLS;
      h[H_INF_PR] = viol; h[H_THETA] = theta; h[H_MU] = mu; h[H_DNORM] = h_dn; h[H_ALPHA_PR] = al; h[H_ALPHA_DU] = az;
      h[H_LS] = n_trials; h[H_KIND] = was_chord ? (reject ? 2 : 1) : 0; h[H_COMPL] = h_cp; h[H_INF_DU] = NAN;
    }
    if (conv || bad || stalled) W.status[b] = conv ? 0 : (bad ? 2 : 1);
    if (conv || bad || stalled || it + 1 >= P.max_iter) {
      W.done[b] = 1;
      W.chord[b] = 0;
      atomicAdd(W.n_active, -1);
    }
    atomicMax(W.n_active + 3, slot + 1);
  }
  if (conv || bad || stalled || it + 1 >= P.max_iter) {
    __syncthreads();
    export_problem(P, W, b, x, conv ? 0 : (bad ? 2 : 1), it + 1, restore ? (improved ? viol : best_viol) : viol);
  }
  if (conv || bad || stalled || it + 1 >= P.max_iter) return;
  const bool chord_off = chord_state == 2 || reject;
  const bool next_chord = P.chord_tol > 0 && !chord_off && al == 1.0 && viol <= P.chord_tol &&
                          (!was_chord || (chord_run < P.chord_max && viol <= P.chord_shrink * prev_viol));
  const int held = (W.held[b] || (P.hold_from > 0 && it + 1 >= P.hold_from && viol <= P.hold_tol)) ? 1 : 0;
  __syncthreads();
  if (tid == 0) W.held[b] = held;
  if (!lin_done) {
    eval_all<true>(P, map, reject ? x : nullptr, g, W.stream + (size_t)b * P.stream_len, evl, (W.trace && it == 1) ? W.trace + ((size_t)b * (P.max_iter + 1) + 72) * 4 : nullptr,
                   held);
  } else if (held != held0) {
    double *Gp = W.stream + (size_t)b * P.stream_len;
    for (int ti = fresh(tid); ti < P.n_terr; ti += nt) {
      const TerrDev TI = P.terr[ti];
      if (TI.d0 >= 0) Gp[TI.d0] = P.hold_weight + TI.ex;
      if (TI.d1 >= 0) Gp[TI.d1] = P.hold_weight + TI.ey;
    }
  }
  __syncthreads();
  KSTAMP(4);
  {
    int rk[KR], ek[KE];
    fresh_rows(rr, rk);
    fresh_rows(er, ek);
#pragma unroll
    for (int k = 0; k < KR; ++k) {
      const int ic = ic_row(k);
      rg[k] = g[rk[k]]; rs[k] = s[rk[k]]; rzl[k] = zl[rk[k]]; rzu[k] = zu[rk[k]];
      rl[k] = P.iq_lo[ic]; ru[k] = P.iq_hi[ic];
    }
#pragma unroll
    for (int k = 0; k < KE; ++k) eg[k] = g[ek[k]];
    double *__restrict__ sigp = W.sig + (size_t)b * m, *__restrict__ wp = W.w + (size_t)b * m, *__restrict__ strm = W.stream + (size_t)b * P.stream_len;
    auto bar_row = [&](bool valid, int r, int sp, int wpos, double l, double u, double sv, double zlv, double zuv, double gv) __attribute__((always_inline)) {
      const bool hl = l > -1e19, hu = u < 1e19;
      const double dl = hl ? sv - l : 1.0, du = hu ? u - sv : 1.0;
      const double zql = zlv / dl, zqu = zuv / du, ml = mu / dl, mq = mu / du;
      const double sg = (hl ? zql : 0.0) + (hu ? zqu : 0.0);
      const double gmu = -(hl ? ml : 0.0) + (hu ? mq : 0.0);
      const double wrv = sg * (gv - sv) + gmu;
      if (valid) {
        sigp[r] = sg;
        wp[r] = wrv;
        strm[sp] = sg;
        strm[wpos] = wrv;
      }
    };
#pragma unroll
    for (int k = 0; k < KE; ++k)
      if (tid + k * nt < P.n_eqw) strm[P.rhs_pos[ek[k]]] = -eg[k];
    for (int i = fresh(tid) + KE * nt; i < P.n_eqw; i += nt) { const int r = P.eq_idx[i]; strm[P.rhs_pos[r]] = -g[r]; }
    int spos[KR], wpos[KR];
#pragma unroll
    for (int k = 0; k < KR; ++k) { spos[k] = P.sig_pos[rk[k]]; wpos[k] = P.w_pos[rk[k]]; }
#pragma unroll
    for (int k = 0; k < KR; ++k) bar_row(tid + k * nt < P.n_iq, rk[k], spos[k], wpos[k], rl[k], ru[k], rs[k], rzl[k], rzu[k], rg[k]);
    for (int i = fresh(tid) + KR * nt; i < P.n_iq; i += nt) {
      const int r = P.iq_idx[i];
      bar_row(true, r, P.sig_pos[r], P.w_pos[r], P.iq_lo[i], P.iq_hi[i], s[r], zl[r], zu[r], g[r]);
    }
  }
  KSTAMP(5);
  if (W.hist) {
    __syncthreads();
    const double du = dual_infeasibility(P, W.stream + (size_t)b * P.stream_len, zl, zu, W.sol + (size_t)b * P.n_stages * PIV, scratch);
    if (tid == 0) W.hist[((size_t)b * (P.max_iter + 1) + it + 1) * HIST_COLS + H_INF_DU] = du;
  }
  if (tid == 0) {
    W.chord[b] = next_chord ? 1 : (chord_off ? 2 : 0);
    W.chord_run[b] = next_chord ? (was_chord ? chord_run + 1 : 1) : 0;
    if (next_chord) atomicAdd(W.n_active + 1, 1);
  }
  if (next_chord) {
    __syncthreads();
    const double *__restrict__ Gs = W.stream + (size_t)b * P.stream_len, *__restrict__ wr = W.w + (size_t)b * m;
    double *__restrict__ rhs = W.rhs + (size_t)b * P.n_unknowns;
    const int NUK = P.n_unknowns, CH = P.rhs_chunk;
    double *accL = evl;
    int *ptrL = (int *)(accL + ((NUK + 1) & ~1));
    double *gvL = (double *)(ptrL + ((NUK + 4) & ~3)), *wvL = gvL + CH;
    for (int p = tid; p <= NUK; p += nt) { ptrL[p] = P.rhs_ptr[p]; if (p < NUK) accL[p] = 0.0; }
    constexpr int SU = 12;
    for (int c0 = 0; c0 < P.n_rhs_ent; c0 += CH) {
      const int c1 = min(c0 + CH, P.n_rhs_ent);
      for (int t = c0 + tid; t < c1; t += SU * nt) {
        int gp[SU], rw[SU];
#pragma unroll
        for (int u = 0; u < SU; ++u) { const int tt = min(t + u * nt, c1 - 1); gp[u] = P.rhs_gpos[tt]; rw[u] = P.rhs_row[tt]; }
        double gv[SU], wv[SU];
#pragma unroll
        for (int u = 0; u < SU; ++u) {
          gv[u] = gp[u] >= 0 ? Gs[max(gp[u], 0)] : 1.0;
          wv[u] = (gp[u] >= 0 ? wr : g)[rw[u]];
        }
#pragma unroll
        for (int u = 0; u < SU; ++u)
          if (t + u * nt < c1) { gvL[t + u * nt - c0] = gv[u]; wvL[t + u * nt - c0] = wv[u]; }
      }
      __syncthreads();
      for (int p = tid; p < NUK; p += nt) {
        const int t0 = max(ptrL[p], c0), t1 = min(ptrL[p + 1], c1);
        if (t0 >= t1) continue;
        double acc = accL[p];
        for (int t = t0; t < t1; t += 8) {
          double gq[8], wq[8];
#pragma unroll
          for (int u = 0; u < 8; ++u) { const int tt = min(t + u, t1 - 1) - c0; gq[u] = gvL[tt]; wq[u] = wvL[tt]; }
#pragma unroll
          for (int u = 0; u < 8; ++u) acc = t + u < t1 ? fma(-gq[u], wq[u], acc) : acc;
        }
        accL[p] = acc;
      }
      __syncthreads();
    }
    for (int p = tid; p < NUK; p += nt) rhs[p] = accL[p];
  }
#ifdef QTOS_STAMPS
  if (tid == 0 && W.trace && it == 1) for (int i = 0; i < 8; ++i) W.trace[((size_t)b * (P.max_iter + 1) + 70) * 4 + i] = (double)ks[i];
#endif
}

__global__ __launch_bounds__(ET) void k_report(DevPlan P, DevWork W, int B) {
  const int b = blockIdx.x;
  if (b >= B) return;
  __shared__ double scratch[ET];
  extern __shared__ double evl[];
  const int n = P.n_vars, m = P.n_cons, tid = threadIdx.x;
  const double *x = W.x + (size_t)b * n;
  double *g = W.g + (size_t)b * m, *Gs = W.stream + (size_t)b * P.stream_len;
  const double *s = W.s + (size_t)b * m, *zl = W.zl + (size_t)b * m, *zu = W.zu + (size_t)b * m;
  const int map = W.map_id ? W.map_id[b] : 0, iters = W.iters[b];
  for (int v = tid; v < n; v += blockDim.x) evl[v] = x[v];
  __syncthreads();
  eval_all<true>(P, map, nullptr, g, Gs, evl, nullptr, W.held[b]);
  __syncthreads();
  double viol, theta;
  infeasibility(P, g, s, scratch, viol, theta);
  double c = 0.0;
  for (int i = tid; i < P.n_iq; i += blockDim.x) { const int r = P.iq_idx[i]; c = fmax(c, compl_row(P.iq_lo[i], P.iq_hi[i], s[r], zl[r], zu[r])); }
  const double compl_ = wg_reduce<1>(c, scratch);
  const double du = dual_infeasibility(P, Gs, zl, zu, iters > 0 ? W.sol + (size_t)b * P.n_stages * PIV : nullptr, scratch);
  if (tid == 0) {
    double *r = W.rep + (size_t)b * REP_COLS;
    r[R_VIOL] = viol; r[R_INF_DU] = du; r[R_COMPL] = compl_;
    r[R_ERR] = (viol == viol && du == du && compl_ == compl_) ? fmax(viol, fmax(du, compl_)) : NAN;
    if (W.hist && iters <= P.max_iter) {
      double *h = W.hist + ((size_t)b * (P.max_iter + 1) + iters) * HIST_COLS;
      if (!(h[H_INF_DU] == h[H_INF_DU])) h[H_INF_DU] = du;
    }
  }
}

struct SampleSpline {
  int n_polys;
  const double *tend;
  const double *dur;
  const int *idx;
};
struct SamplePlan {
  SampleSpline lin, ang, eem[NEE], eef[NEE];
  int n_vars;
  double T;
};

template <bool EXACT_START = false>
__device__ inline void sample_spline(const SampleSpline &S, const double *x, double t, int deriv, double out[3]) {
  int lo = 0, hi = S.n_polys - 1;
  while (lo < hi) {
    const int mid = (lo + hi) >> 1;
    if (S.tend[mid] >= t - 1e-10) hi = mid; else lo = mid + 1;
  }
  const int k = lo;
  const double T = S.dur[k];
  double tau = t - (S.tend[k] - T);
  if (EXACT_START) tau -= S.tend[S.n_polys + k];
  double w[4];
  const double T2 = T * T, T3 = T2 * T, t2 = tau * tau, t3 = t2 * tau;
  if (deriv == 0) {
    w[0] = 1 - 3 * t2 / T2 + 2 * t3 / T3; w[1] = tau - 2 * t2 / T + t3 / T2;
    w[2] = 3 * t2 / T2 - 2 * t3 / T3; w[3] = -t2 / T + t3 / T2;
  } else {
    w[0] = -6 * tau / T2 + 6 * t2 / T3; w[1] = 1 - 4 * tau / T + 3 * t2 / T2;
    w[2] = 6 * tau / T2 - 6 * t2 / T3; w[3] = -2 * tau / T + 3 * t2 / T2;
// ... 892 lines not shown
```

quadruped-trajectory-optimization-stack_amd/csrc/model.hpp:

```cpp
#pragma once
#include <algorithm>
#include <array>
#include <cmath>
#include <cstdint>
#include <cstring>
#include <cstdlib>
#include <string>
#include <vector>

#include "../../include/qtos_planner.h"

namespace qtos {

constexpr int NEE = QTOS_NEE;
constexpr double BIG = 1e20;

struct VecIn {
  double w[4];
  int var[12];
};

struct DynInst {
  VecIn r, a, th, thd, thdd, p[NEE], f[NEE];
  int row0, goff, ncol, in_kkt;
  short c_lin[12], c_ang[12], c_p[NEE][12], c_f[NEE][12];
};
struct RomInst {
  VecIn r, th, p;
  int row0, goff, ncol, ee;
  short c_lin[12], c_ang[12], c_p[12];
};
struct TerrInst {
  int vx, vy, vz, row, goff, ncol, in_kkt;
  short cx, cy, cz, pad;
};
struct ForceInst {
  int vf[3], vsx, vsy, row0, goff, ncol;
  short cf[3], csx, csy, pad;
};
struct LinRow {
  int row, n;
  int var[8];
  double coef[8];
};
constexpr int DYN_LOC = 54;
constexpr int ROM_LOC = 18;
struct ColDesc {
  int inst, gbase, ncol;
  short kind, dim;
  double w0, w1, w2;
};
struct LinTerm1 { int pos, off; double a; };
struct LinTerm3 { int pos, off[3]; double a[3]; };
struct PackedTerm1 { unsigned pos; unsigned short off, ai; };
struct PackedTerm3 { unsigned pos; unsigned short off[3], ai[3]; };
struct Block {
  int kind;
  int m, n, row0, goff, gstatic, col_off, pad;
};
struct IqRow {
  int goff;
  int n;
  int col_off;
  int row;
};
struct SwTask {
  int goff;
  int n;
  int row;
  int c16_off;
  int cpos_off;
  int pad[3];
};
struct InitDesc {
  int set;
  int dim;
  int is_vel;
  int fix_src;
  double frac;
};

struct Spline {
  int n_polys = 0;
  std::vector<double> dur;
  std::vector<std::array<int, 6>> idx;

  void locate(double t, int &k, double &tau) const {
    const double eps = 1e-10;
    double acc = 0;
    int id = n_polys - 1;
    for (int i = 0; i < n_polys; ++i) {
      acc += dur[i];
      if (acc >= t - eps) { id = i; break; }
    }
    double tl = t;
    for (int i = 0; i < id; ++i) tl -= dur[i];
    k = id;
    tau = tl;
  }
  double node_time(int node) const {
    double t = 0;
    for (int i = 0; i < node; ++i) t += dur[i];
    return t;
  }
};

inline void hermite_weights(double T, double t, int deriv, double w[4]) {
  const double T2 = T * T, T3 = T2 * T, t2 = t * t, t3 = t2 * t;
  if (deriv == 0) {
    w[0] = 1 - 3 * t2 / T2 + 2 * t3 / T3;
    w[1] = t - 2 * t2 / T + t3 / T2;
    w[2] = 3 * t2 / T2 - 2 * t3 / T3;
    w[3] = -t2 / T + t3 / T2;
  } else if (deriv == 1) {
    w[0] = -6 * t / T2 + 6 * t2 / T3;
    w[1] = 1 - 4 * t / T + 3 * t2 / T2;
    w[2] = 6 * t / T2 - 6 * t2 / T3;
    w[3] = -2 * t / T + 3 * t2 / T2;
  } else {
    w[0] = -6 / T2 + 12 * t / T3;
    w[1] = -4 / T + 6 * t / T2;
    w[2] = 6 / T2 - 12 * t / T3;
    w[3] = -2 / T + 6 * t / T2;
  }
}

inline void bspline_ders(const std::vector<double> &U, int i, double t, double ders[3][4]) {
  const int p = 3;
  double ndu[4][4], left[4], right[4], a[2][4];
// ... 812 lines not shown
```

quadruped-trajectory-optimization-stack_amd/csrc/qtos_planner.hip:

```cpp
#include <hip/hip_runtime.h>

#include <cstdio>
#include <cstdlib>
#include <cstring>
#include <atomic>
#include <chrono>
#include <cmath>
#include <string>
#include <map>
#include <memory>
#include <vector>

#include "kernels.hpp"
#include "kkt2.hpp"
#include "kkt3.hpp"
#include "kkt5.hpp"
#include "csv_writer.hpp"

using namespace qtos;

#define HIPCHK(p, call)                                                                       \
  do {                                                                                        \
    hipError_t e_ = (call);                                                                   \
    if (e_ != hipSuccess) {                                                                   \
// ... 310 lines not shown
    auto at = [&](int e) { return (unsigned)cpos[c0 + e] & 0xffffu; };
    for (int q = 0; q < 4; ++q)
      for (int u = 0; u < SW_RU; u += 2) {
        const int e0 = std::max(std::min(q + 4 * u, n4 - 4 + q), 0), e1 = std::max(std::min(q + 4 * (u + 1), n4 - 4 + q), 0);
        c16.push_back((int)(at(std::min(e0, b.n - 1)) | (at(std::min(e1, b.n - 1)) << 16)));
      }
    {
      const int r0 = std::min(n4, b.n - 1), r1 = std::min(n4 + 1, b.n - 1), r2 = std::min(n4 + 2, b.n - 1);
      c16.push_back((int)(at(r0) | (at(r1) << 16)));
      c16.push_back((int)at(r2));
      c16.push_back(0); c16.push_back(0);
    }
    for (int r = 0; r < b.m; ++r) by_stage[mn / PIV].push_back({b.goff + r * b.n, b.n, b.row0 + r, k0, c0, {0, 0, 0}});
  }
  if ((size_t)NS * PIV > 65535) ok = false;
  const SwTask none = {0, 4, -1, 0, 0, {0, 0, 0}};
  int step = 0;
  auto round_of = [&](const SwTask *t, int cnt) {
    for (int i = 0; i < SW_ROUND; ++i) tasks.push_back(i < cnt ? t[i] : none);
    ++step;
  };
  for (int u = NS - 1; u >= 0 && ok; --u) {
    while (step < NS - u) round_of(nullptr, 0);
    for (size_t i = 0; i < by_stage[u].size(); i += SW_ROUND) round_of(by_stage[u].data() + i, (int)std::min<size_t>(SW_ROUND, by_stage[u].size() - i));
  }
  const int nstep = ((NS + SWD - 1) / SWD) * SWD;
  while (step < nstep) round_of(nullptr, 0);
  if (cpos.empty()) cpos.push_back(0);
  while (c16.size() < 20) c16.push_back(0);
  if (S.env.debug) {
    size_t mx = 0, tot = 0;
    for (auto &v : by_stage) { mx = std::max(mx, v.size()); tot += v.size(); }
    fprintf(stderr, "qtos: sweep ds: %d rounds for %d stages (chain %d steps), %zu rows, most in a stage %zu; rows by stage:", step, NS, nstep, tot, mx);
    for (auto &v : by_stage) fprintf(stderr, " %zu", v.size());
    fprintf(stderr, "\n");
  }
  return ok ? step : 0;
}

static int create_planner(const QtosParams *params, int max_batch, int device, const QtosEnv &env0, int order_rule, QtosPlanner **out, Analysis *pre = nullptr) {
  if (!params || !out || max_batch < 1 || max_batch >= (1 << 24)) return -1;
  *out = nullptr;
  QtosPlanner *p = new QtosPlanner();
  p->device = device;
  p->max_batch = max_batch;
  p->env = env0;
  const QtosEnv &env = p->env;
  p->spec_pattern = env.spec_pattern != 0;
  if (choose_kernel(*params, env, p->kkt, *p, order_rule, pre)) { delete p; return -1; }
  const HostModel &M = p->M;
  const Symbolic &S = p->S;
  int ndev = 0;
  if (hipGetDeviceCount(&ndev) != hipSuccess || ndev <= device) {
    fprintf(stderr, "qtos: no HIP device %d (found %d) -- the planner has no CPU fallback\n", device, ndev);
    delete p;
    return -2;
  }
  int rc = 0;
#define TRY(x) do { if ((rc = (x))) { fprintf(stderr, "qtos: %s\n", p->err.c_str()); qtos_planner_destroy(p); return rc; } } while (0)
  {
    hipError_t e = hipSetDevice(device);
    if (e != hipSuccess) { delete p; return -2; }
  }
  DevPlan &D = p->dp;
  std::memset(&D, 0, sizeof(D));
  D.n_vars = M.n_vars; D.n_cons = M.n_cons; D.n_stages = S.n_stages; D.front = S.front;
  D.n_sol = M.n_sol; D.n_rec = (int)M.rec_var.size();
  {
    std::vector<char> is_rec(M.n_sol, 0);
    for (int v : M.rec_var) is_rec[v] = 1;
    for (int c : M.rec_col)
      if (c >= 0 && is_rec[c]) { p->err = "reduced base: a recovered node value is the source of another"; fprintf(stderr, "qtos: %s\n", p->err.c_str()); delete p; return -1; }
  }
  TRY(p->upload(M.rec_var, &D.rec_var)); TRY(p->upload(M.rec_col, &D.rec_col)); TRY(p->upload(M.rec_w, &D.rec_w));
  D.n_coef = M.reduce_base ? M.n_coef : 0; D.n_pz = (int)M.pz_var.size();
  TRY(p->upload(M.pc_var, &D.pc_var)); TRY(p->upload(M.pc_w, &D.pc_w));
  D.n_psw = (int)M.psw_var.size();
  TRY(p->upload(M.psw_var, &D.psw_var)); TRY(p->upload(M.psw_src, &D.psw_src)); TRY(p->upload(M.psw_w, &D.psw_w));
  TRY(p->upload(M.pz_var, &D.pz_var)); TRY(p->upload(M.pz_col, &D.pz_col)); TRY(p->upload(M.pz_w, &D.pz_w));
  D.n_dyn = (int)M.dyn.size(); D.n_rom = (int)M.rom.size(); D.n_terr = (int)M.terr.size();
  D.n_force = (int)M.force.size(); D.n_lin = (int)M.linrow.size(); D.n_blocks = (int)M.blocks.size();
  TRY(p->upload(M.dyn, &D.dyn)); TRY(p->upload(M.rom, &D.rom));
  {
    auto flat = [&](const void *inst0, size_t inst_bytes, size_t n_inst, int n_vec, const i4_t **var, const d2_t **wa, const d2_t **wb) {
      std::vector<i4_t> v;
      std::vector<d2_t> a, b;
      for (size_t i = 0; i < n_inst; ++i)
        for (int k = 0; k < n_vec; ++k) {
          const VecIn &in = ((const VecIn *)((const char *)inst0 + i * inst_bytes))[k];
          for (int d = 0; d < 3; ++d) {
            v.push_back(i4_t{in.var[d], in.var[3 + d], in.var[6 + d], in.var[9 + d]});
            a.push_back(d2_t{in.w[0], in.w[1]});
            b.push_back(d2_t{in.w[2], in.w[3]});
          }
        }
      int rc2 = p->upload(v, var);
      if (!rc2) rc2 = p->upload(a, wa);
      if (!rc2) rc2 = p->upload(b, wb);
      return rc2;
    };
    static_assert(DYN_VIN == 39 && ROM_VIN == 9, "13 / 3 input vectors of three components");
    TRY(flat(M.dyn.data(), sizeof(DynInst), M.dyn.size(), 13, &D.pre_dyn_var, &D.pre_dyn_wa, &D.pre_dyn_wb));
    TRY(flat(M.rom.data(), sizeof(RomInst), M.rom.size(), 3, &D.pre_rom_var, &D.pre_rom_wa, &D.pre_rom_wb));
  }
  TRY(p->upload(M.force, &D.force)); TRY(p->upload(M.linrow, &D.lin));
  {
    std::map<unsigned long long, int> idx_of;
    std::vector<double> coefs;
    bool fits = true;
    auto ci = [&](double a) {
      unsigned long long bits;
      std::memcpy(&bits, &a, 8);
      auto it = idx_of.find(bits);
      if (it == idx_of.end()) { it = idx_of.emplace(bits, (int)coefs.size()).first; coefs.push_back(a); }
      return (unsigned short)it->second;
    };
    auto off16 = [&](int off) { if (off < 0 || off > 65535) fits = false; return (unsigned short)off; };
    std::vector<PackedTerm1> d1, r1;
    std::vector<PackedTerm3> d3;
    for (const LinTerm1 &t : S.dyn_t1) d1.push_back({(unsigned)t.pos, off16(t.off), ci(t.a)});
    for (const LinTerm1 &t : S.rom_t1) r1.push_back({(unsigned)t.pos, off16(t.off), ci(t.a)});
    for (const LinTerm3 &t : S.dyn_t3)
      d3.push_back({(unsigned)t.pos, {off16(t.off[0]), off16(t.off[1]), off16(t.off[2])}, {ci(t.a[0]), ci(t.a[1]), ci(t.a[2])}});
    if (!fits || coefs.size() > 65535) {
      p->err = "Jacobian entry lists exceed the packed format (16-bit offsets / coefficient indices)";
      fprintf(stderr, "qtos: %s\n", p->err.c_str());
      qtos_planner_destroy(p);
      return -4;
    }
    D.n_lin_coef = (int)coefs.size();
    TRY(p->upload(d1, &D.dyn_t1)); TRY(p->upload(d3, &D.dyn_t3)); TRY(p->upload(r1, &D.rom_t1)); TRY(p->upload(coefs, &D.lin_coef));
  }
  TRY(p->upload(S.dyn_t1_off, &D.dyn_t1_off)); TRY(p->upload(S.dyn_t3_off, &D.dyn_t3_off));
  D.n_rom_t1 = (int)S.rom_t1.size();
  D.dyn_chunk = M.dyn_chunk;
  D.rom_chunk = S.rom_chunk;
  TRY(p->upload(S.rom_t1_off, &D.rom_t1_off));
  TRY(p->upload(S.amask, &D.amask));
  TRY(p->upload(S.amask2, &D.amask2));
  TRY(p->upload(S.nxt_pack, &D.nxt_pack));
  TRY(p->upload(S.ctab, &D.ctab));
  TRY(p->upload(S.rtab, &D.rtab));
  TRY(p->upload(S.rhs_ptr, &D.rhs_ptr)); TRY(p->upload(S.rhs_gpos, &D.rhs_gpos)); TRY(p->upload(S.rhs_row, &D.rhs_row));
  TRY(p->upload(S.kx_ptr, &D.kx_ptr)); TRY(p->upload(S.kx_col, &D.kx_col)); TRY(p->upload(S.kx_pos, &D.kx_pos));
  D.n_unknowns = S.n_unknowns;
  D.chord_tol = M.P.chord_tol;
  D.chord_max = M.P.chord_max > 0 ? M.P.chord_max : 1;
  D.chord_shrink = M.P.chord_shrink > 0 ? M.P.chord_shrink : 1.0 / 3.0;
  D.n_cells = S.n_cells;
  D.n_cont = S.n_continuation();
  D.table = nullptr; D.tab_dx = D.tab_dy = nullptr; D.tab_ndx = D.tab_ndy = 0;
  D.off_lin = M.off_lin; D.off_ang = M.off_ang;
  for (int e = 0; e < NEE; ++e) D.off_eem[e] = M.off_eem[e];
  TRY(p->upload(S.cont, &D.cont));
  {
    std::vector<int> dpos_of_var(M.n_sol, -1);
    for (int i = 0; i < (int)S.pack_src.size(); ++i)
      if ((S.pack_src[i] >> 28) == 5) {
        const int u = S.piv_unknown[S.pack_src[i] & 0x0fffffff];
        if (u >= 0 && u < M.n_sol) dpos_of_var[u] = i;
      }
    std::vector<TerrDev> td;
    for (const TerrInst &t : M.terr) {
      TerrDev d = {t.vx, t.vy, t.vz, t.row, -1, -1, -1, -1, -1, 0, 0.0, 0.0};
      if (t.in_kkt) {
        const bool stance = M.row_kind[t.row] == 1;
        auto pos = [&](int c) { return c < 0 ? -1 : (stance ? S.eq_pos[t.goff + c] : t.goff + c); };
        d.px = pos(t.cx); d.py = pos(t.cy); d.pz = pos(t.cz);
        if (M.P.hold_from > 0 && stance) {
          d.d0 = dpos_of_var[t.vx]; d.d1 = dpos_of_var[t.vy];
          d.ex = M.sol_diag[t.vx] - M.P.delta_x; d.ey = M.sol_diag[t.vy] - M.P.delta_x;
        }
      }
      td.push_back(d);
    }
    TRY(p->upload(td, &D.terr));
    D.hold_from = M.P.hold_from;
    D.spec_jac = env.spec_jac;
    D.hold_weight = M.P.hold_weight > 0 ? M.P.hold_weight : 1e6;
    D.hold_tol = M.P.hold_tol;
  }
  TRY(p->upload(M.blocks, &D.blocks)); TRY(p->upload(M.block_cols, &D.block_cols));
  {
    std::vector<IqRow> rows;
    for (const Block &b : M.blocks)
      if (b.kind == 1)
        for (int r = 0; r < b.m; ++r) rows.push_back({b.goff + r * b.n, b.n, b.col_off, b.row0 + r});
    D.n_iq_rows = (int)rows.size();
    TRY(p->upload(rows, &D.iq_rows));
  }
  {
    std::vector<SwTask> tasks;
    std::vector<int> cpos, c16;
    D.sw_steps = build_sweep_tasks(M, S, tasks, cpos, c16);
    const bool ok = D.sw_steps > 0;
    D.sw_on = ok && D.n_iq_rows > 0 && S.front / PIV < SW_W0 && env.sweep_ds != 0;
    TRY(p->upload(tasks, &D.sw_tasks)); TRY(p->upload(cpos, &D.sw_cpos)); TRY(p->upload(c16, &D.sw_c16));
  }
  {
    std::vector<int> iq, eq;
    std::vector<double> lo, hi;
    for (int r = 0; r < M.n_cons; ++r) {
      if (M.row_kind[r] == 2) { iq.push_back(r); lo.push_back(M.con_lo[r]); hi.push_back(M.con_hi[r]); }
      else if (M.row_kind[r] == 1) eq.push_back(r);
    }
    D.n_iq = (int)iq.size(); D.n_eqw = (int)eq.size();
    TRY(p->upload(iq, &D.iq_idx)); TRY(p->upload(eq, &D.eq_idx));
    TRY(p->upload(lo, &D.iq_lo)); TRY(p->upload(hi, &D.iq_hi));
  }
  TRY(p->upload(M.g_static, &D.g_static));
  TRY(p->upload(S.piv_slot, &D.piv_slot)); TRY(p->upload(S.piv_unknown, &D.piv_unknown));
  TRY(p->upload(S.piv_diag, &D.piv_diag)); TRY(p->upload(S.stages, &D.stages));
  TRY(p->upload(S.eq_entries, &D.eq_entries)); TRY(p->upload(S.eq_rhs, &D.eq_rhs));
  TRY(p->upload(S.iq_blocks, &D.iq_blocks)); TRY(p->upload(S.iq_slots, &D.iq_slots));
  TRY(p->upload(M.con_lo, &D.con_lo)); TRY(p->upload(M.con_hi, &D.con_hi));
  TRY(p->upload(M.row_kind, &D.row_kind)); TRY(p->upload(M.init, &D.init));
  TRY(p->upload(M.node_time, &D.var_time));
  D.max_stage_g = S.max_stage_g;
  TRY(p->upload(S.srec, &D.srec)); TRY(p->upload(S.srec_off, &D.srec_off));
  TRY(p->upload(S.pack_src, &D.pack_src)); TRY(p->upload(S.drec_off, &D.drec_off));
  TRY(p->upload(S.diag_pos, &D.diag_pos));
  TRY(p->upload(S.pair_groups, &D.pair_groups));
  TRY(p->upload(S.eq_pos, &D.eq_pos)); TRY(p->upload(S.rhs_pos, &D.rhs_pos));
  TRY(p->upload(S.sig_pos, &D.sig_pos)); TRY(p->upload(S.w_pos, &D.w_pos));
  D.max_srec = S.max_srec; D.max_drec = S.max_drec; D.stream_len = (int)S.pack_src.size();
  D.mass = M.P.mass; D.gravity = M.P.gravity; D.mu_fric = M.P.mu; D.f_max = M.P.f_max; D.T = M.T;
  for (int i = 0; i < 9; ++i) D.Ib[i] = M.P.inertia_b[i];
  for (int e = 0; e < NEE; ++e)
    for (int d = 0; d < 3; ++d) D.nominal[e][d] = M.P.nominal_stance[e][d];
  D.tol = M.P.tol; D.mu_init = M.P.mu_init; D.mu_min = M.P.mu_min; D.delta_x = M.P.delta_x;
  D.mu_superlinear = M.P.mu_superlinear != 0;
  D.eps_dual = M.P.eps_dual; D.max_iter = M.P.max_iter; D.stall_iters = M.P.stall_iters; D.stall_alpha = M.P.stall_alpha;
  D.slack_push = M.P.slack_push > 0 ? M.P.slack_push : 0.01;
  D.warm_slack_push = M.P.warm_slack_push > 0 ? M.P.warm_slack_push : 0.01;
  D.terrain_mode = M.P.terrain_mode;
  D.g_doubles = S.g_doubles;
  D.panel_stride = (long long)S.n_stages * (S.front + 1) * PIV;
  const int F = S.front;
  p->kkt_lds = kkt_lds_bytes(p->kkt, S);
  D.kron_lds_off = 0;
  if (env.debug) fprintf(stderr, "qtos: Kronecker assembly %s (kkt3 %d, most blocks in a record %d)\n", S.kron ? "on" : "off", (int)(p->kkt == Kkt::kkt3), S.max_kblocks);
  if (S.kron) {
    D.kron_lds_off = (int)((p->kkt_lds + 15) & ~(size_t)15);
    p->kkt_lds = (size_t)D.kron_lds_off + sizeof(double) * Symbolic::KRON_SM * (size_t)S.max_kblocks;
  }
  if (p->kkt == Kkt::kkt5 && F > 128) D.sw_on = 0;
  if (D.sw_on) {
    const size_t need = (p->kkt == Kkt::kkt5 ? kkt5_sweep_base_bytes(F, S.n_stages) : kkt2_sweep_base_bytes(F, S.n_stages)) + sweep_ds_lds_bytes(S.n_stages, D.sw_steps);
    if (need > LDS_LIMIT || chord_lds_bytes(S.n_stages, D.sw_steps) > 96 * 1024) D.sw_on = 0;
    else p->kkt_lds = std::max(p->kkt_lds, need);
  }
  p->kkt_threads = p->kkt == Kkt::kkt5 ? KT5 : KT2;
  const int max_front = 208;
  if (p->kkt != Kkt::kkt5 && (S.max_drec > 2 * 2 * KT || S.max_srec > 3 * 4 * KT || F > max_front || (S.pack_src.size() & 1))) {
    p->err = "stage record exceeds the prefetch registers";
    fprintf(stderr, "qtos: stage records too long (%d doubles, %d ints) or front %d > %d\n", S.max_drec, S.max_srec, F, max_front);
    qtos_planner_destroy(p);
    return -4;
  }
  if (env.debug) fprintf(stderr, "qtos: front %d, k_kkt LDS %zu B\n", F, p->kkt_lds);
  if (p->kkt_lds > LDS_LIMIT) {
    p->err = "front too large for LDS";
    fprintf(stderr, "qtos: front %d needs %zu B of LDS\n", F, p->kkt_lds);
    qtos_planner_destroy(p);
    return -4;
  }
  {
    switch (p->kkt) {
      case Kkt::kkt5: p->kkt_fn = kkt5_kernel(F); break;
      case Kkt::kkt3: p->kkt_fn = kkt3_kernel(F); break;
      case Kkt::kkt2: p->kkt_fn = kkt2_kernel(F, D.n_cont > 0, S.kron); break;
    }
    p->chord_fn = chord_kernel(F);
    if (!p->kkt_fn) { p->err = "no k_kkt instantiation for this front size"; qtos_planner_destroy(p); return -4; }
    hipError_t e = hipFuncSetAttribute((const void *)p->kkt_fn, hipFuncAttributeMaxDynamicSharedMemorySize, (int)p->kkt_lds);
    if (e != hipSuccess) { p->err = std::string("hipFuncSetAttribute: ") + hipGetErrorString(e); fprintf(stderr, "qtos: %s\n", p->err.c_str()); qtos_planner_destroy(p); return -2; }
    if (p->chord_fn && D.sw_on) {
      e = hipFuncSetAttribute((const void *)p->chord_fn, hipFuncAttributeMaxDynamicSharedMemorySize, (int)chord_lds_bytes(S.n_stages, D.sw_steps));
      if (e != hipSuccess) { p->err = std::string("hipFuncSetAttribute: ") + hipGetErrorString(e); fprintf(stderr, "qtos: %s\n", p->err.c_str()); qtos_planner_destroy(p); return -2; }
    }
  }
  p->eval_lds = sizeof(double) * (((size_t)M.n_sol + 1) / 2 * 2 + std::max((size_t)DYN_LOC * D.dyn_chunk, (size_t)ROM_LOC * D.rom_chunk) +
                                  std::max((size_t)DYN_VIN * D.dyn_chunk, (size_t)ROM_VIN * D.rom_chunk));
  D.coef_in_lds = p->eval_lds + sizeof(double) * (size_t)D.n_lin_coef <= 150 * 1024;
  if (D.coef_in_lds) p->eval_lds += sizeof(double) * (size_t)D.n_lin_coef;
  {
    D.n_rhs_ent = (int)S.rhs_gpos.size();
    const size_t nuk = (size_t)S.n_unknowns, fixed = ((nuk + 1) & ~(size_t)1) + ((nuk + 4) & ~(size_t)3) / 2;
    const size_t room = 150 * 1024 / sizeof(double) > fixed ? (150 * 1024 / sizeof(double) - fixed) / (2 * (size_t)ET) : 0;
    D.rhs_chunk = (int)std::max<size_t>(1, std::min<size_t>(std::min<size_t>((D.n_rhs_ent + ET - 1) / ET, 12), room)) * ET;
    p->eval_lds = std::max(p->eval_lds, (fixed + 2 * (size_t)D.rhs_chunk) * sizeof(double));
  }
  if (p->eval_lds > 150 * 1024) {
    p->err = "too many dynamics knots for the LDS scratch";
    fprintf(stderr, "qtos: evaluation kernels need %zu B of LDS\n", p->eval_lds);
    qtos_planner_destroy(p);
    return -4;
  }
  for (const void *fn : {(const void *)k_start, (const void *)k_step, (const void *)k_debug_eval})
    if (hipFuncSetAttribute(fn, hipFuncAttributeMaxDynamicSharedMemorySize, (int)p->eval_lds) != hipSuccess) { qtos_planner_destroy(p); return -2; }
  if (hipFuncSetAttribute((const void *)k_probe, hipFuncAttributeMaxDynamicSharedMemorySize, (int)probe_lds_bytes(1, PP_GRID)) != hipSuccess) { qtos_planner_destroy(p); return -2; }
  SamplePlan &SP = p->sp;
  std::memset(&SP, 0, sizeof(SP));
  SP.n_vars = M.n_vars; SP.T = M.T;
  TRY(upload_spline(p, M.lin, &SP.lin)); TRY(upload_spline(p, M.ang, &SP.ang));
  for (int e = 0; e < NEE; ++e) { TRY(upload_spline(p, M.eem[e], &SP.eem[e])); TRY(upload_spline(p, M.eef[e], &SP.eef[e])); }
  TRY(p->alloc(&p->d_sp, 1));
  HIPCHK(p, hipMemcpy(p->d_sp, &SP, sizeof(SP), hipMemcpyHostToDevice));
  DevWork &W = p->wk;
  std::memset(&W, 0, sizeof(W));
  const size_t Bm = (size_t)max_batch, n = M.n_vars, m = M.n_cons;
  TRY(p->alloc(&W.x, Bm * n)); TRY(p->alloc(&W.dx, Bm * (size_t)M.n_sol));
  TRY(p->alloc(&W.g, Bm * m)); TRY(p->alloc(&W.gt, Bm * m)); TRY(p->alloc(&W.s, Bm * m));
  TRY(p->alloc(&W.zl, Bm * m)); TRY(p->alloc(&W.zu, Bm * m)); TRY(p->alloc(&W.ds, Bm * m));
  TRY(p->alloc(&W.dzl, Bm * m)); TRY(p->alloc(&W.dzu, Bm * m)); TRY(p->alloc(&W.sig, Bm * m));
  TRY(p->alloc(&W.w, Bm * m));
  TRY(p->alloc(&W.panel, Bm * (size_t)D.panel_stride));
  TRY(p->alloc(&W.stream, Bm * (size_t)S.pack_src.size() + 64));
  {
    std::vector<double> one(S.pack_src.size(), 0.0);
    for (size_t i = 0; i < S.const_pos.size(); ++i) one[S.const_pos[i]] = S.const_val[i];
    for (size_t b = 0; b < Bm; ++b)
      HIPCHK(p, hipMemcpy(W.stream + b * one.size(), one.data(), one.size() * sizeof(double), hipMemcpyHostToDevice));
  }
  TRY(p->alloc(&W.mu, Bm)); TRY(p->alloc(&W.viol, Bm));
  TRY(p->alloc(&W.best_viol, Bm)); TRY(p->alloc(&W.best_it, Bm)); TRY(p->alloc(&W.xbest, Bm * n));
  TRY(p->alloc(&W.held, Bm));
#ifdef QTOS_STAMPS
  if (M.P.max_iter < 79) { p->err = "diagnostic build (QTOS_STAMPS) parks its stamps in trace rows 16..79: create the planner with max_iter >= 79"; fprintf(stderr, "qtos: %s\n", p->err.c_str()); qtos_planner_destroy(p); return -1; }
#endif
  TRY(p->alloc(&W.trace, Bm * (size_t)(M.P.max_iter + 1) * 4));
  TRY(p->alloc(&W.hist, Bm * (size_t)(M.P.max_iter + 1) * HIST_COLS)); TRY(p->alloc(&W.rep, Bm * (size_t)REP_COLS));
  TRY(p->alloc(&W.status, Bm)); TRY(p->alloc(&W.iters, Bm)); TRY(p->alloc(&W.done, Bm));
  TRY(p->alloc(&W.n_active, 4 * 4));
  TRY(p->alloc(&W.chord, Bm));
  TRY(p->alloc(&W.chord_run, Bm));
  TRY(p->alloc(&W.jam, Bm));
  TRY(p->alloc(&W.rhs, Bm * (size_t)S.n_unknowns));
  TRY(p->alloc(&W.minv, Bm * (size_t)S.n_stages * PIV * PIV));
  TRY(p->alloc(&W.sol, Bm * (size_t)S.n_stages * PIV)); TRY(p->alloc(&W.sol0, Bm * (size_t)S.n_stages * PIV));
  TRY(p->alloc(&W.dx0, Bm * (size_t)M.n_sol)); TRY(p->alloc(&W.ur, Bm * m));
  TRY(p->alloc(&p->d_start, Bm * QTOS_START_DOUBLES)); TRY(p->alloc(&p->d_goal, Bm * 3));
  TRY(p->alloc(&p->d_nodes, Bm * n)); TRY(p->alloc(&p->d_warm, Bm * n)); TRY(p->alloc(&p->d_map, Bm));
  if (hipStreamCreateWithFlags(&p->own_stream, hipStreamNonBlocking) != hipSuccess) { qtos_planner_destroy(p); return -2; }
  if (hipMalloc(&p->d_totals, 2 * sizeof(long long)) != hipSuccess || hipMemset(p->d_totals, 0, 2 * sizeof(long long)) != hipSuccess) { qtos_planner_destroy(p); return -3; }
  p->last_stream = p->own_stream;
  p->max_slots = 2 * M.P.max_iter + 2;
  {
    int cus = 256;
    if (hipDeviceGetAttribute(&cus, hipDeviceAttributeMultiprocessorCount, device) != hipSuccess || cus < 1) cus = 256;
    p->lane_chunk = cus;
    const int want = env.lanes;
    const int n_lanes = std::max(1, std::min(want, (max_batch + cus - 1) / cus));
    p->lanes.resize(n_lanes);
    if (hipEventCreateWithFlags(&p->ev_in, hipEventDisableTiming) != hipSuccess) { qtos_planner_destroy(p); return -2; }
    for (int j = 0; j < n_lanes; ++j) {
      QtosPlanner::Lane &L = p->lanes[j];
      if (hipHostMalloc((void **)&L.h_active, 4 * sizeof(int) * ((size_t)p->max_slots + 1), hipHostMallocMapped) != hipSuccess) { qtos_planner_destroy(p); return -3; }
      if (hipHostGetDevicePointer((void **)&L.h_active_dev, L.h_active, 0) != hipSuccess) { qtos_planner_destroy(p); return -2; }
      L.was_kkt.assign(p->max_slots + 1, 0);
      L.was_chord.assign(p->max_slots + 1, 0);
      L.d_n_active = W.n_active + 4 * j;
      if (j > 0 && hipStreamCreateWithFlags(&L.own, hipStreamNonBlocking) != hipSuccess) { qtos_planner_destroy(p); return -2; }
      if (hipStreamCreateWithFlags(&L.side, hipStreamNonBlocking) != hipSuccess) { qtos_planner_destroy(p); return -2; }
      if (hipEventCreateWithFlags(&L.ev_fork, hipEventDisableTiming) != hipSuccess || hipEventCreateWithFlags(&L.ev_join, hipEventDisableTiming) != hipSuccess ||
          hipEventCreateWithFlags(&L.ev_done, hipEventDisableTiming) != hipSuccess) { qtos_planner_destroy(p); return -2; }
      L.ev.resize(5 * (size_t)p->max_slots + 3);
      for (auto &e : L.ev)
        if (hipEventCreate(&e) != hipSuccess) { qtos_planner_destroy(p); return -2; }
    }
  }
#undef TRY
  *out = p;
  return 0;
}

// ... 523 lines not shown
  out[0] = tot; out[1] = start; out[2] = solve; out[3] = step; out[4] = gaps;
  out[5] = L.last_launches; out[6] = L.spec; out[7] = L.n_informed;
  out[8] = (double)p->n_pattern_calls; out[9] = (double)p->n_pattern_misses;
  if (n_out >= 14) { out[10] = kkt_s; out[11] = kkt_n; out[12] = chord_s; out[13] = chord_n; }
  return 0;
}

static_assert(HIST_COLS == QTOS_HIST_COLS && H_INF_DU == QTOS_H_INF_DU && H_KIND == QTOS_H_KIND, "history layout: kernels.hpp and the header");

int qtos_set_report(QtosPlanner *p, int on) {
  if (!p) return -1;
  if (p->call_open || p->busy.load()) { p->err = "qtos_set_report: a call is open (the flag is latched per call at submit)"; return -5; }
  p->report = on != 0;
  return 0;
}

int qtos_plan_report(QtosPlanner *p, int b, QtosReport *out, double *rows, int max_rows) {
  if (!p || !out || b < 0 || (rows && max_rows < 0)) return -1;
  if (!p->last_report || b >= p->last_B) { p->err = "qtos_plan_report: the last call ran without the report, or b is outside it"; return -6; }
  if (p->call_open) return -5;
  HIPCHK(p, hipSetDevice(p->device));
  HIPCHK(p, hipStreamSynchronize(p->last_stream));
  const int stride = p->M.P.max_iter + 1;
  int st = 0, it = 0;
  double rep[REP_COLS];
  std::vector<double> h((size_t)stride * HIST_COLS);
  HIPCHK(p, hipMemcpy(&st, p->wk.status + b, sizeof(int), hipMemcpyDeviceToHost));
  HIPCHK(p, hipMemcpy(&it, p->wk.iters + b, sizeof(int), hipMemcpyDeviceToHost));
  HIPCHK(p, hipMemcpy(rep, p->wk.rep + (size_t)b * REP_COLS, sizeof(rep), hipMemcpyDeviceToHost));
  HIPCHK(p, hipMemcpy(h.data(), p->wk.hist + (size_t)b * stride * HIST_COLS, h.size() * sizeof(double), hipMemcpyDeviceToHost));
  const int n_rows = std::min(it + 1, stride);
  std::memset(out, 0, sizeof(*out));
  out->status = st; out->iterations = it; out->n_rows = n_rows;
  out->n_con_evals = 1; out->n_jac_evals = 1;
  for (int i = 1; i < n_rows; ++i) {
    const double *r = h.data() + (size_t)i * HIST_COLS;
    out->n_con_evals += (int)r[H_LS];
    if (r[H_KIND] == 0) out->n_factorizations++; else out->n_chord_solves++;
    if (i + 1 < n_rows) out->n_jac_evals++;
  }
  out->constraint_violation = rep[R_VIOL]; out->dual_infeasibility = rep[R_INF_DU];
  out->complementarity = rep[R_COMPL]; out->nlp_error = rep[R_ERR];
  if (rows && max_rows > 0) std::memcpy(rows, h.data(), (size_t)std::min(n_rows, max_rows) * HIST_COLS * sizeof(double));
  return n_rows;
}

int qtos_analyze_counts(const QtosParams *params, long long *counts, int n) {
  if (!params || !counts || n < 0) return -1;
  QtosParams full = *params;
  full.reduce_base = 0; full.reduce_swing = 0;
  HostModel M;
  if (M.build(full)) { fprintf(stderr, "qtos: %s\n", M.err.c_str()); return -1; }
  long long nz[2] = {0, 0};
  for (const Block &blk : M.blocks)
    for (int r = 0; r < blk.m; ++r) {
      const int row = blk.row0 + r, k = M.con_lo[row] == M.con_hi[row] ? 0 : 1;
      for (int a = 0; a < blk.n; ++a) nz[k] += M.is_free(M.block_cols[blk.col_off + a]) ? 1 : 0;
    }
  const int k = std::min(n, 2);
  for (int i = 0; i < k; ++i) counts[i] = nz[i];
  return k;
}

int qtos_set_kernel_events(QtosPlanner *p, int on) {
  if (!p) return -1;
  p->per_kernel_events = on != 0;
  return 0;
}

int qtos_set_pattern_speculation(QtosPlanner *p, int on) {
  if (!p) return -1;
  p->spec_pattern = on != 0;
  if (!on) { p->pat.clear(); p->obs_prev.clear(); }
  return 0;
}

int qtos_env(const QtosPlanner *p, char *buf, int n) {
  if (!p || !buf || n < 1) return -1;
  const std::string d = p->env.describe();
  snprintf(buf, (size_t)n, "%s", d.c_str());
  return (int)d.size();
}

int qtos_last_timing_chord(QtosPlanner *p, double *chord_seconds, int *chord_launches) {
  if (!p) return -1;
  if (!p->per_kernel_events) { p->err = "per-kernel events are off (qtos_set_kernel_events)"; return -1; }
  HIPCHK(p, hipSetDevice(p->device));
  HIPCHK(p, hipEventSynchronize(p->lanes[0].ev[1]));
  double t = 0;
  int nl = 0;
  for (int j = 0; j < p->lanes_used; ++j) {
    const QtosPlanner::Lane &L = p->lanes[j];
    for (int i = 0; i < L.last_launches; ++i) {
      if (!L.was_chord[i]) continue;
      float ms = 0;
      HIPCHK(p, hipEventElapsedTime(&ms, L.ev[4 + 5 * i], L.ev[5 + 5 * i]));
      t += ms * 1e-3;
      ++nl;
    }
  }
  if (chord_seconds) *chord_seconds = t;
  if (chord_launches) *chord_launches = nl;
  return 0;
}

int qtos_sample_csv_device(QtosPlanner *p, int B, const double *d_nodes, const double *d_t0, double hz,
                           int n_rows, double *d_rows_out, void *stream_) {
  if (!p || B < 1 || !d_nodes || !d_t0 || !d_rows_out || n_rows < 1 || !(hz > 0)) return -1;
  HIPCHK(p, hipSetDevice(p->device));
  dim3 grid((n_rows + 255) / 256, B);
  hipLaunchKernelGGL(k_sample, grid, dim3(256), 0, (hipStream_t)stream_, p->sp, d_nodes, d_t0, hz, n_rows, d_rows_out, B);
  HIPCHK(p, hipGetLastError());
  return 0;
}

int qtos_write_csv(const char *path, const double *rows, int n_rows, int n_threads) {
  return write_csv_file(path, rows, n_rows, QTOS_CSV_COLS, n_threads);
}

int qtos_sample_csv(QtosPlanner *p, int B, const double *nodes, const double *t0, double hz, int n_rows, double *rows_out) {
  if (!p || B < 1 || !nodes || !t0 || !rows_out) return -1;
  HIPCHK(p, hipSetDevice(p->device));
  double *d_nodes = nullptr, *d_t0 = nullptr, *d_rows = nullptr;
  const size_t n = p->M.n_vars, rows_bytes = (size_t)B * n_rows * QTOS_CSV_COLS * sizeof(double);
  HIPCHK(p, hipMalloc((void **)&d_nodes, (size_t)B * n * sizeof(double)));
  HIPCHK(p, hipMalloc((void **)&d_t0, B * sizeof(double)));
  HIPCHK(p, hipMalloc((void **)&d_rows, rows_bytes));
  HIPCHK(p, hipMemcpy(d_nodes, nodes, (size_t)B * n * sizeof(double), hipMemcpyHostToDevice));
  HIPCHK(p, hipMemcpy(d_t0, t0, B * sizeof(double), hipMemcpyHostToDevice));
  int rc = qtos_sample_csv_device(p, B, d_nodes, d_t0, hz, n_rows, d_rows, nullptr);
  if (!rc) {
    hipError_t e = hipMemcpy(rows_out, d_rows, rows_bytes, hipMemcpyDeviceToHost);
    if (e != hipSuccess) rc = -2;
  }
  (void)hipFree(d_nodes); (void)hipFree(d_t0); (void)hipFree(d_rows);
  return rc;
}

__global__ __launch_bounds__(256) void k_shift_warm(DevPlan P, SamplePlan S, const double *prev, const double *offset,
                                                    const double *start, const double *goal, const int *map_id, double *out, int B) {
  const int b = blockIdx.x;
  if (b >= B) return;
  const double *x = prev + (size_t)b * P.n_vars, *st = start + (size_t)b * QTOS_START_DOUBLES, *gl = goal + (size_t)b * 3;
  const int map = map_id ? map_id[b] : 0;
  const double off = offset[b];
  for (int v = threadIdx.x; v < P.n_vars; v += blockDim.x) {
    const InitDesc I = P.init[v];
    double val;
    if (I.fix_src >= 0) val = I.fix_src < 24 ? st[I.fix_src] : (I.fix_src < 26 ? gl[I.fix_src - 24] : 0.0);
    else {
      const double t = off + P.var_time[v];
      if (t <= S.T + 1e-9) {
        SampleSpline sp = S.lin;
        if (I.set == 1) sp = S.ang;
#pragma unroll
        for (int e = 0; e < NEE; ++e) {
          if (I.set == 2 + e) sp = S.eem[e];
          if (I.set == 6 + e) sp = S.eef[e];
        }
        double o3[3];
        sample_spline<true>(sp, x, fmin(t, S.T), I.is_vel, o3);
        val = o3[I.dim];
      } else val = straight_line_value(P, I, st, gl, map);
    }
    out[(size_t)b * P.n_vars + v] = val;
  }
// ... 1121 lines not shown
```

quadruped-trajectory-optimization-stack_amd/csrc/symbolic.hpp:

```cpp
#pragma once
#include <algorithm>
#include <array>
#include <cstdio>
#include <cstdlib>
#include <cmath>
#include <cstring>
#include <map>
#include <set>
#include <numeric>
#include <vector>

#include "env.hpp"
#include "model.hpp"

namespace qtos {

constexpr int PIV = 16;

constexpr int kkt_pick_nu(int ntile) {
  if (ntile == 21) return 12;
  int best = 14, best_t = (ntile + 13) / 14;
  for (int nu = 14; nu >= 8; --nu) {
    const int t = (ntile + nu - 1) / nu;
    if (t < best_t || (t == best_t && nu * t - ntile <= best * best_t - ntile)) { best = nu; best_t = t; }
// ... 71 lines not shown
  std::vector<int> kx_ptr, kx_col, kx_pos;
  int cell_mode = 2;
  std::vector<int> rtab;
  std::vector<unsigned> amask;
  std::vector<unsigned> amask2;
  std::vector<int> nxt_pack;
  std::vector<int> eq_pos, rhs_pos, sig_pos, w_pos, const_pos;
  std::vector<double> const_val;
  int max_srec = 0, max_drec = 0;
  long long g_doubles = 0;
  long long algorithmic_bytes = 0, flops = 0, envelope = 0;
  int max_active = 0;
  std::string err;

  std::vector<LinTerm1> dyn_t1, rom_t1;
  std::vector<LinTerm3> dyn_t3;
  std::vector<int> dyn_t1_off, dyn_t3_off;
  std::vector<int> rom_t1_off;
  int rom_chunk = 1;
  void build_linear_terms(HostModel &M) {
    const int n_dyn = (int)M.dyn.size(), n_ch = std::max(1, (n_dyn + 127) / 128);
    M.dyn_chunk = std::max(1, (n_dyn + n_ch - 1) / n_ch);
    std::vector<std::vector<LinTerm1>> t1(n_ch);
    std::vector<std::vector<LinTerm3>> t3(n_ch);
    auto skew = [](int i, int d, int &k, double &sgn) {
      k = 3 - i - d;
      sgn = ((d - i + 3) % 3 == 1) ? -1.0 : 1.0;
    };
    for (const ColDesc &c : M.dyn_cols) {
      const int ch = c.inst / M.dyn_chunk, base = (c.inst - ch * M.dyn_chunk) * DYN_LOC, d = c.dim;
      for (int i = 0; i < 6; ++i) {
        const int pos = eq_pos[c.gbase + i * c.ncol];
        double cst = 0.0;
        bool is_const = true;
        if (i < 3 && c.kind == 1) {
          LinTerm3 t;
          t.pos = pos;
          t.off[0] = base + 3 * i + d; t.off[1] = base + 9 + 3 * i + d; t.off[2] = base + 18 + 3 * i + d;
          t.a[0] = c.w0; t.a[1] = c.w1; t.a[2] = c.w2;
          t3[ch].push_back(t);
          is_const = false;
        } else if (i < 3 && i != d) {
          int k; double sgn;
          skew(i, d, k, sgn);
          const int vec = c.kind == 0 ? 27 : (c.kind < 6 ? 30 + 3 * (c.kind - 2) : 42 + 3 * (c.kind - 6));
          t1[ch].push_back({pos, base + vec + k, (c.kind == 0 ? -sgn : sgn) * c.w0});
          is_const = false;
        } else if (i >= 3 && i - 3 == d) {
          if (c.kind == 0) cst = M.P.mass * c.w1;
          else if (c.kind >= 6) cst = -c.w0;
        }
        if (is_const) { const_pos.push_back(pos); const_val.push_back(cst); }
      }
    }
    dyn_t1.clear(); dyn_t3.clear(); dyn_t1_off.assign(1, 0); dyn_t3_off.assign(1, 0);
    for (int ch = 0; ch < n_ch; ++ch) {
      std::sort(t1[ch].begin(), t1[ch].end(), [](const LinTerm1 &a, const LinTerm1 &b) { return a.pos < b.pos; });
      std::sort(t3[ch].begin(), t3[ch].end(), [](const LinTerm3 &a, const LinTerm3 &b) { return a.pos < b.pos; });
      dyn_t1.insert(dyn_t1.end(), t1[ch].begin(), t1[ch].end());
      dyn_t3.insert(dyn_t3.end(), t3[ch].begin(), t3[ch].end());
      dyn_t1_off.push_back((int)dyn_t1.size());
      dyn_t3_off.push_back((int)dyn_t3.size());
    }
    const int n_rom = (int)M.rom.size(), n_chr = std::max(1, (n_rom + 511) / 512);
    rom_chunk = std::max(1, (n_rom + n_chr - 1) / n_chr);
    std::vector<std::vector<LinTerm1>> r1(n_chr);
    for (const ColDesc &c : M.rom_cols) {
      const int ch = c.inst / rom_chunk, base = (c.inst - ch * rom_chunk) * ROM_LOC, d = c.dim;
      for (int i = 0; i < 3; ++i) {
        const int pos = c.gbase + i * c.ncol;
        if (c.kind == 1) r1[ch].push_back({pos, base + 9 + 3 * i + d, c.w0});
        else r1[ch].push_back({pos, base + 3 * d + i, (c.kind == 2 ? 1.0 : -1.0) * c.w0});
      }
    }
    rom_t1.clear();
    rom_t1_off.assign(1, 0);
    for (int ch = 0; ch < n_chr; ++ch) {
      std::sort(r1[ch].begin(), r1[ch].end(), [](const LinTerm1 &a, const LinTerm1 &b) { return a.pos < b.pos; });
      rom_t1.insert(rom_t1.end(), r1[ch].begin(), r1[ch].end());
      rom_t1_off.push_back((int)rom_t1.size());
    }
  }

  static constexpr int SHDR_INTS = 8;
  int REC_MAX_DOUBLES = 2048, REC_MAX_INTS = 6144;
  int rec_cap_ints = 0;
  std::vector<int> cont;
  KMeta kron_meta(const HostModel &M, int bi) const {
    KMeta K;
    const Block &b = M.blocks[bi];
    if (b.kind != 1 || b.m != 3 || b.n > 32 || M.reduce_swing) return K;
    int inst = -1;
    for (size_t k = 0; k < M.rom.size(); ++k)
      if (M.rom[k].goff == bi) { inst = (int)k; break; }
    if (inst < 0) return K;
    const RomInst &I = M.rom[inst];
    const HostModel::BaseIn &Bi = M.rom_sol[inst];
    double alpha[32];
    int kind[32];
    for (int c = 0; c < b.n; ++c) { alpha[c] = 0.0; kind[c] = -1; K.d[c] = 0; K.mu[c] = 0; K.grp[c] = 0; }
    auto add = [&](const short cmap[12], const VecIn &in, int kd, double sgn) {
      for (int sidx = 0; sidx < 4; ++sidx)
        for (int d = 0; d < 3; ++d) {
          const int c = cmap[3 * sidx + d];
          if (c < 0 || c >= b.n) continue;
          if (kind[c] >= 0 && (kind[c] != kd || K.d[c] != d)) { kind[c] = 99; continue; }
          kind[c] = kd; K.d[c] = (unsigned char)d; K.mu[c] = kd == 1 ? 1 : 0;
          alpha[c] += sgn * in.w[sidx];
        }
    };
    add(I.c_lin, Bi.r, 0, -1.0);
    add(I.c_ang, Bi.th, 1, 1.0);
    add(I.c_p, I.p, 2, 1.0);
    for (int c = 0; c < b.n; ++c)
      if (kind[c] < 0 || kind[c] == 99 || alpha[c] == 0.0) return K;
    double galpha[12];
    int gkind[12];
    for (int c = 0; c < b.n; ++c) {
      int g = -1;
      for (int j = 0; j < K.n_grp; ++j)
        if (gkind[j] == kind[c] && galpha[j] == alpha[c]) { g = j; break; }
      if (g < 0) {
        if (K.n_grp == 12) return K;
        g = K.n_grp++;
        gkind[g] = kind[c]; galpha[g] = alpha[c];
      }
      K.grp[c] = (unsigned char)g;
    }
    double ralpha[2] = {0.0, 0.0};
    for (int i = 0; i < 6; ++i) K.rep[i] = -1;
    for (int mu = 0; mu < 2; ++mu) {
      int best = -1;
      for (int g = 0; g < K.n_grp; ++g) {
        if ((gkind[g] == 1 ? 1 : 0) != mu) continue;
        bool have[3] = {false, false, false};
        for (int c = 0; c < b.n; ++c)
          if (K.grp[c] == g) have[K.d[c]] = true;
        if (have[0] && have[1] && have[2] && (best < 0 || std::fabs(galpha[g]) > std::fabs(galpha[best]))) best = g;
      }
      bool any = false;
      for (int g = 0; g < K.n_grp; ++g) any |= (gkind[g] == 1 ? 1 : 0) == mu;
      if (best < 0) { if (any) return K; continue; }
      ralpha[mu] = galpha[best];
      for (int c = 0; c < b.n; ++c)
        if (K.grp[c] == best) K.rep[3 * mu + K.d[c]] = c;
    }
    int repg[2] = {-1, -1};
    for (int mu = 0; mu < 2; ++mu)
      if (K.rep[3 * mu] >= 0) repg[mu] = K.grp[K.rep[3 * mu]];
    int renum[12], n_tab = 0;
    for (int g = 0; g < K.n_grp; ++g) renum[g] = (g == repg[0] || g == repg[1]) ? 15 : n_tab++;
    if (n_tab > 10) return K;
    for (int g = 0; g < 12; ++g) K.rho[g] = 0.0;
    for (int g = 0; g < K.n_grp; ++g)
      if (renum[g] != 15) K.rho[renum[g]] = galpha[g] / ralpha[gkind[g] == 1 ? 1 : 0];
    for (int c = 0; c < b.n; ++c) K.grp[c] = (unsigned char)renum[K.grp[c]];
    K.n_grp = n_tab;
    for (int c = 0; c < 32; ++c) K.alpha[c] = c < b.n ? alpha[c] : 0.0;
    K.ok = true;
    return K;
  }
  double check_kron(int *n_blocks) const {
    double worst = 0.0;
    unsigned rng = 12345u;
    auto rnd = [&]() { rng = rng * 1664525u + 1013904223u; return ((rng >> 8) & 0xffff) / 65536.0 - 0.5; };
    *n_blocks = 0;
// ... 957 lines not shown
```

Baseline: 109,800.

## Evaluate dynamics and ROM constraints jointly in one LDS pass when they fit

Adds a 'joint' evaluation schedule that, when all dynamics and ROM instances fit in LDS, runs both prepasses and both evaluations in a single phase, then writes all Jacobian terms at once. This removes the per-chunk barriers and the serial dyn-then-ROM phases. When the coefficient table no longer fits alongside the inputs, it is loaded late into the region the inputs occupied. The schedule is enabled by default, and the ROM term offsets are rebased into a merged term array. It also adds analysis and query APIs, plus small register-uniformity hints (fresh/fresh_uniform).

```diff
diff --git a/include/qtos_planner.h b/include/qtos_planner.h
--- a/include/qtos_planner.h
+++ b/include/qtos_planner.h
@@ -206,6 +206,9 @@
 int qtos_set_speculation(QtosPlanner *p, int max_blind_iterations);
 int qtos_set_pattern_speculation(QtosPlanner *p, int on);
 int qtos_env(const QtosPlanner *p, char *buf, int n);
+int qtos_eval_schedule(const QtosPlanner *p);
+#define QTOS_EVAL_LAYOUT_FIELDS 18
+int qtos_analyze_eval_layout(const QtosParams *params, long long *out, int n);
 
 int qtos_last_timing(QtosPlanner *p, double *kkt_seconds, int *kkt_launches, double *total_seconds,
                      int *iterations);
diff --git a/quadruped-trajectory-optimization-stack_amd/capi.py b/quadruped-trajectory-optimization-stack_amd/capi.py
--- a/quadruped-trajectory-optimization-stack_amd/capi.py
+++ b/quadruped-trajectory-optimization-stack_amd/capi.py
@@ -260,6 +260,7 @@
     "qtos_path_goal", "qtos_path_goal_device", "qtos_path_plan", "qtos_path_plan_device",
     "qtos_probe", "qtos_probe_device", "qtos_probe_stamp", "qtos_probe_stamp_device",
     "qtos_terrain_env", "qtos_terrain_env_device", "qtos_set_heightfields_device",
+    "qtos_eval_schedule", "qtos_analyze_eval_layout",
 ]
 
 _lib = None
@@ -375,6 +376,9 @@
         u64p = C.POINTER(C.c_uint64)
         lib.qtos_terrain_env.argtypes = [vp, C.POINTER(QtosTerrainEnv), dp, ip, u64p, ip, dp, dp, ip]
         lib.qtos_terrain_env_device.argtypes = [vp, C.POINTER(QtosTerrainEnv)] + [vp] * 8
+    if hasattr(lib, "qtos_eval_schedule"):
+        lib.qtos_eval_schedule.argtypes = [vp]
+        lib.qtos_analyze_eval_layout.argtypes = [C.POINTER(QtosParams), C.POINTER(C.c_longlong), C.c_int]
     if hasattr(lib, "qtos_set_heightfields_device"):
         lib.qtos_set_heightfields_device.argtypes = [vp, C.c_int, vp, C.c_int, C.c_int, C.c_double, C.c_double, C.c_double, vp]
     _lib = lib
@@ -463,6 +467,22 @@
     return int(c[0]), int(c[1])
 
 
+EVAL_LAYOUT_FIELDS = ("schedule", "joint", "bytes", "limit", "coef_in_lds", "packed_fits", "loc_dyn", "loc_rom", "vin_dyn", "vin_rom",
+                      "coef", "end", "n_dyn", "n_rom", "n_coef", "n_rom_t1", "rom_off_min", "rom_off_max")
+
+
+def analyze_eval_layout(cfg):
+    lib = load()
+    if not hasattr(lib, "qtos_analyze_eval_layout"):
+        return None
+    p = params_from_config(cfg)
+    n = len(EVAL_LAYOUT_FIELDS)
+    a = (C.c_longlong * n)()
+    if lib.qtos_analyze_eval_layout(C.byref(p), a, n) != n:
+        raise ValueError("qtos_analyze_eval_layout failed")
+    return {k: int(a[i]) for i, k in enumerate(EVAL_LAYOUT_FIELDS)}
+
+
 def analyze_kernel(cfg):
     lib = load()
     p = params_from_config(cfg)
@@ -924,6 +944,11 @@
         self._chk(self.lib.qtos_debug_initial_guess(self.h, start.shape[0], _dp(start), _dp(goal), _ip(mid), _dp(out)), "initial_guess")
         return out
 
+    def eval_schedule(self):
+        if not hasattr(self.lib, "qtos_eval_schedule"):
+            return 0
+        return int(self.lib.qtos_eval_schedule(self.h))
+
     def kkt_kernel(self):
         buf = C.create_string_buffer(64)
         self.lib.qtos_kkt_kernel.argtypes = [C.c_void_p, C.c_char_p, C.c_int]
diff --git a/quadruped-trajectory-optimization-stack_amd/csrc/env.hpp b/quadruped-trajectory-optimization-stack_amd/csrc/env.hpp
--- a/quadruped-trajectory-optimization-stack_amd/csrc/env.hpp
+++ b/quadruped-trajectory-optimization-stack_amd/csrc/env.hpp
@@ -12,6 +12,7 @@
   int short_stages = -1;
   int sweep_ds = 1;
   int spec_jac = 1;
+  int eval_joint = 1;
   int spec_pattern = 1;
   int kron = 0;
   int order = -1;
@@ -29,6 +30,7 @@
     if (num("QTOS_NO_SHORT_STAGES", 0) != 0) e.short_stages = 0;
     e.sweep_ds = num("QTOS_SWEEP_DS", 1) != 0;
     e.spec_jac = num("QTOS_SPEC_JAC", 1) != 0;
+    e.eval_joint = std::max(0, std::min(2, num("QTOS_EVAL_JOINT", 1)));
     e.spec_pattern = num("QTOS_SPEC_PATTERN", 1) != 0;
     e.kron = num("QTOS_KRON", 0) != 0;
     e.place = num("QTOS_PLACE", 0);
@@ -40,9 +42,9 @@
   }
   std::string describe() const {
     char b[320];
-    snprintf(b, sizeof(b), "QTOS_KKT=%d QTOS_LANES=%d QTOS_SHORT_STAGES=%s QTOS_SWEEP_DS=%d QTOS_SPEC_JAC=%d QTOS_SPEC_PATTERN=%d QTOS_KRON=%d QTOS_PLACE=%d QTOS_ORDER=%s QTOS_DEBUG_SYMBOLIC=%d",
+    snprintf(b, sizeof(b), "QTOS_KKT=%d QTOS_LANES=%d QTOS_SHORT_STAGES=%s QTOS_SWEEP_DS=%d QTOS_SPEC_JAC=%d QTOS_SPEC_PATTERN=%d QTOS_KRON=%d QTOS_PLACE=%d QTOS_ORDER=%s QTOS_DEBUG_SYMBOLIC=%d QTOS_EVAL_JOINT=%d",
              kkt, lanes, short_stages < 0 ? "unset" : (short_stages ? "1" : "0"), sweep_ds, spec_jac, spec_pattern, kron, place,
-             order < 0 ? "unset" : (order == 2 ? "2" : order ? "1" : "0"), debug);
+             order < 0 ? "unset" : (order == 2 ? "2" : order ? "1" : "0"), debug, eval_joint);
     return b;
   }
 };
diff --git a/quadruped-trajectory-optimization-stack_amd/csrc/kernels.hpp b/quadruped-trajectory-optimization-stack_amd/csrc/kernels.hpp
--- a/quadruped-trajectory-optimization-stack_amd/csrc/kernels.hpp
+++ b/quadruped-trajectory-optimization-stack_amd/csrc/kernels.hpp
@@ -42,7 +42,8 @@
   const double *lin_coef;
   int n_lin_coef, coef_in_lds;
   const int *dyn_t1_off, *dyn_t3_off;
-  int n_rom_t1;
+  int n_rom_t1, n_dyn_t1, n_dyn_t3;
+  int eval_joint, ev_loc, ev_loc_rom, ev_vin, ev_vin_rom, ev_coef, ev_coef_late;
   int rom_chunk;
   const int *rom_t1_off;
   int dyn_chunk;
@@ -367,7 +368,7 @@
 #ifndef TERM3_UNROLL
 #define TERM3_UNROLL 8
 #endif
-__device__ inline void write_terms1(const PackedTerm1 *T, int i0, int i1, const double *loc, const double *coef, double *G) {
+__device__ __forceinline__ void write_terms1(const PackedTerm1 *T, int i0, int i1, const double *loc, const double *coef, double *G) {
   const int nt = blockDim.x;
   constexpr int UN = TERM1_UNROLL;
   for (int i = i0 + threadIdx.x; i < i1; i += UN * nt) {
@@ -379,7 +380,7 @@
       if (i + u * nt < i1) G[t[u].pos] = coef[t[u].ai] * loc[t[u].off];
   }
 }
-__device__ inline void write_terms3(const PackedTerm3 *T, int i0, int i1, const double *loc, const double *coef, double *G) {
+__device__ __forceinline__ void write_terms3(const PackedTerm3 *T, int i0, int i1, const double *loc, const double *coef, double *G) {
   const int nt = blockDim.x;
   constexpr int UN = TERM3_UNROLL;
   for (int i = i0 + threadIdx.x; i < i1; i += UN * nt) {
@@ -460,9 +461,12 @@
 }
 
 __device__ __forceinline__ int eval_loc_offset(int n_vars) { return (n_vars + 1) & ~1; }
-constexpr int DYN_VIN = 39, ROM_VIN = 9;
 __device__ __forceinline__ int fresh(int v) {
   asm volatile("" : "+v"(v));
+  return v;
+}
+__device__ __forceinline__ double fresh_uniform(double v) {
+  asm volatile("" : "+s"(v));
   return v;
 }
 __device__ __forceinline__ void wg_lds_barrier() { asm volatile("s_waitcnt lgkmcnt(0)\n\ts_barrier" ::: "memory"); }
@@ -474,6 +478,25 @@
 #else
 #define EVAL_BARRIER() __syncthreads()
 #endif
+
+template <bool JAC>
+__device__ __forceinline__ void dyn_item(const DevPlan &P, const DynInst *D, int it, int cnt, int cpad, const double *vin, double *loc, double *g) {
+  const int what = JAC ? it / cpad : 0, i = it - what * cpad;
+  if (i >= cnt) return;
+  const DynInst &I = D[i];
+  const double *vi = vin + (size_t)i * DYN_VIN, *th = vi + 6, *thd = vi + 9, *thdd = vi + 12;
+  const Trig tg = trig_of(th);
+  if (JAC) {
+    double *li = loc + (size_t)i * DYN_LOC;
+    if (what == 0) eval_dyn<true>(P, I, vi, g, li, th, thd, thdd, tg);
+    else if (what == 1) eval_dyn_pass<0>(P, I, li, th, thd, thdd, tg);
+    else if (what == 2) eval_dyn_pass<1>(P, I, li, th, thd, thdd, tg);
+    else eval_dyn_pass<2>(P, I, li, th, thd, thdd, tg);
+  } else {
+    eval_dyn<false>(P, I, vi, g, nullptr, th, thd, thdd, tg);
+  }
+}
+
 template <bool JAC>
 __device__ inline void eval_all(const DevPlan &P, int map, const double *xg, double *g, double *G, double *lds, double *dbg = nullptr,
                                 int hold = -1) {
@@ -485,63 +508,51 @@
 #else
 #define ESTAMP() do {} while (0)
 #endif
-  double *x = lds, *loc = lds + eval_loc_offset(P.n_vars);
-  double *vin = loc + max(DYN_LOC * P.dyn_chunk, ROM_LOC * P.rom_chunk);
-  double *coef_lds = vin + max(DYN_VIN * P.dyn_chunk, ROM_VIN * P.rom_chunk);
-  const double *coef = P.coef_in_lds ? coef_lds : P.lin_coef;
+  double *x = lds, *coef_lds = lds + P.ev_coef;
+  const bool joint = P.eval_joint != 0;
   if (xg)
     for (int v = fresh(tid); v < P.n_vars; v += nt) x[v] = xg[v];
-  if (JAC && P.coef_in_lds)
+  if (JAC && P.coef_in_lds && !P.ev_coef_late)
     for (int v = fresh(tid); v < P.n_lin_coef; v += nt) coef_lds[v] = P.lin_coef[v];
   EVAL_BARRIER();
-  for (int c0 = 0, ch = 0; c0 < P.n_dyn; c0 += P.dyn_chunk, ++ch) {
-    const int cnt = min(P.dyn_chunk, P.n_dyn - c0);
-    if (c0) EVAL_BARRIER();
-    vec_prepass(P.pre_dyn_var + c0 * DYN_VIN, P.pre_dyn_wa + c0 * DYN_VIN, P.pre_dyn_wb + c0 * DYN_VIN, cnt * DYN_VIN, x, vin);
+  double *loc = lds + P.ev_loc, *loc_rom = lds + P.ev_loc_rom, *vin = lds + P.ev_vin, *vin_rom = lds + P.ev_vin_rom;
+  const double *coef = P.coef_in_lds ? coef_lds : P.lin_coef;
+  const int npd = joint ? 1 : (P.n_dyn + P.dyn_chunk - 1) / P.dyn_chunk, npr = joint ? 0 : (P.n_rom + P.rom_chunk - 1) / P.rom_chunk;
+  for (int ps = 0; ps < npd + npr; ++ps) {
+    int d0 = 0, dcnt = 0, r0 = 0, rcnt = 0;
+    if (joint) {
+      dcnt = P.n_dyn; rcnt = P.n_rom;
+    } else if (ps < npd) {
+      d0 = ps * P.dyn_chunk; dcnt = min(P.dyn_chunk, P.n_dyn - d0);
+    } else {
+      r0 = (ps - npd) * P.rom_chunk; rcnt = min(P.rom_chunk, P.n_rom - r0);
+    }
+    if (ps) EVAL_BARRIER();
+    {
+      const int i0 = dcnt ? d0 * DYN_VIN : P.n_dyn * DYN_VIN + r0 * ROM_VIN;
+      vec_prepass(P.pre_dyn_var + i0, P.pre_dyn_wa + i0, P.pre_dyn_wb + i0, dcnt * DYN_VIN + rcnt * ROM_VIN, x, dcnt ? vin : vin_rom);
+    }
+    EVAL_BARRIER();
+    if (dcnt) ESTAMP();
+    {
+      const int cpad = (dcnt + 63) & ~63, nd = dcnt ? (JAC ? 4 : 1) * cpad : 0;
+      for (int it = tid; it < nd; it += nt) dyn_item<JAC>(P, P.dyn + d0, it, dcnt, cpad, vin, loc, g);
+      int i = tid - nd % nt;
+      if (i < 0) i += nt;
+      for (; i < rcnt; i += nt) eval_rom<JAC>(P, P.rom[r0 + i], vin_rom + (size_t)i * ROM_VIN, g, JAC ? loc_rom + (size_t)i * ROM_LOC : nullptr);
+    }
+    if (!JAC) { ESTAMP(); continue; }
+    if (joint) break;
     EVAL_BARRIER();
     ESTAMP();
-    if (JAC) {
-      const int cpad = (cnt + 63) & ~63;
-      for (int it = tid; it < 4 * cpad; it += nt) {
-        const int what = it / cpad, i = it - what * cpad;
-        if (i >= cnt) continue;
-        double *li = loc + (size_t)i * DYN_LOC;
-        const DynInst &I = P.dyn[c0 + i];
-        const double *vi = vin + (size_t)i * DYN_VIN, *th = vi + 6, *thd = vi + 9, *thdd = vi + 12;
-        const Trig tg = trig_of(th);
-        if (what == 0) eval_dyn<true>(P, I, vi, g, li, th, thd, thdd, tg);
-        else if (what == 1) eval_dyn_pass<0>(P, I, li, th, thd, thdd, tg);
-        else if (what == 2) eval_dyn_pass<1>(P, I, li, th, thd, thdd, tg);
-        else eval_dyn_pass<2>(P, I, li, th, thd, thdd, tg);
-      }
+    if (dcnt) {
+      write_terms1(P.dyn_t1, P.dyn_t1_off[ps], P.dyn_t1_off[ps + 1], loc, coef, G);
+      write_terms3(P.dyn_t3, P.dyn_t3_off[ps], P.dyn_t3_off[ps + 1], loc, coef, G);
       EVAL_BARRIER();
-      ESTAMP();
-      write_terms1(P.dyn_t1, P.dyn_t1_off[ch], P.dyn_t1_off[ch + 1], loc, coef, G);
-      write_terms3(P.dyn_t3, P.dyn_t3_off[ch], P.dyn_t3_off[ch + 1], loc, coef, G);
-      EVAL_BARRIER();
-      ESTAMP();
     } else {
-      for (int i = tid; i < cnt; i += nt) {
-        const DynInst &I = P.dyn[c0 + i];
-        const double *vi = vin + (size_t)i * DYN_VIN, *th = vi + 6, *thd = vi + 9, *thdd = vi + 12;
-        eval_dyn<false>(P, I, vi, g, nullptr, th, thd, thdd, trig_of(th));
-      }
-      ESTAMP();
-    }
-  }
-  for (int c0 = 0, ch = 0; c0 < P.n_rom; c0 += P.rom_chunk, ++ch) {
-    const int cnt = min(P.rom_chunk, P.n_rom - c0);
-    EVAL_BARRIER();
-    vec_prepass(P.pre_rom_var + c0 * ROM_VIN, P.pre_rom_wa + c0 * ROM_VIN, P.pre_rom_wb + c0 * ROM_VIN, cnt * ROM_VIN, x, vin);
-    EVAL_BARRIER();
-    for (int i = tid; i < cnt; i += nt) eval_rom<JAC>(P, P.rom[c0 + i], vin + (size_t)i * ROM_VIN, g, JAC ? loc + (size_t)i * ROM_LOC : nullptr);
-    if (!JAC) ESTAMP();
-    if (JAC) {
-      EVAL_BARRIER();
-      ESTAMP();
-      write_terms1(P.rom_t1, P.rom_t1_off[ch], P.rom_t1_off[ch + 1], loc, coef, G);
-      ESTAMP();
-    }
+      write_terms1(P.rom_t1, P.rom_t1_off[ps - npd], P.rom_t1_off[ps - npd + 1], loc, coef, G);
+    }
+    ESTAMP();
   }
   {
     const int rt = nt - 1 - tid;
@@ -571,6 +582,24 @@
     }
   }
   ESTAMP();
+  if (JAC && joint) {
+    if (P.ev_coef_late) {
+      constexpr int UN = 8;
+      double c[UN];
+      const int n = P.n_lin_coef, v0 = fresh(tid);
+#pragma unroll
+      for (int u = 0; u < UN; ++u) c[u] = P.lin_coef[min(v0 + u * nt, n - 1)];
+      EVAL_BARRIER();
+#pragma unroll
+      for (int u = 0; u < UN; ++u)
+        if (v0 + u * nt < n) coef_lds[v0 + u * nt] = c[u];
+      for (int v = v0 + UN * nt; v < n; v += nt) coef_lds[v] = P.lin_coef[v];
+    }
+    EVAL_BARRIER();
+    write_terms1(P.dyn_t1, 0, P.n_dyn_t1 + P.n_rom_t1, loc, coef, G);
+    write_terms3(P.dyn_t3, 0, P.n_dyn_t3, loc, coef, G);
+    ESTAMP();
+  }
 }
 
 #ifndef QTOS_ET
@@ -1341,7 +1370,7 @@
 #pragma unroll
     for (int k = 0; k < KE; ++k) egt[k] = gv[ek[k]];
     th = l1_rows(rgt, egt, st_, dst, gv, al);
-    if (th <= (1.0 - 1e-4 * al) * th0 || th < 1e-9) { lin_done = spec && ls == 0; break; }
+    if (th <= (1.0 - 1e-4 * al) * th0 || th < fresh_uniform(1e-9)) { lin_done = spec && ls == 0; break; }
     if (ls < 5) al *= 0.5;
   }
   KSTAMP(2);
@@ -1496,7 +1525,7 @@
                    held);
   } else if (held != held0) {
     double *Gp = W.stream + (size_t)b * P.stream_len;
-    for (int ti = fresh(tid); ti < P.n_terr; ti += nt) {
+    for (int ti = fresh(tid); ti < P.n_terr; ti += fresh(nt)) {
       const TerrDev TI = P.terr[ti];
       if (TI.d0 >= 0) Gp[TI.d0] = P.hold_weight + TI.ex;
       if (TI.d1 >= 0) Gp[TI.d1] = P.hold_weight + TI.ey;
@@ -1560,15 +1589,15 @@
     __syncthreads();
     const double *__restrict__ Gs = W.stream + (size_t)b * P.stream_len, *__restrict__ wr = W.w + (size_t)b * m;
     double *__restrict__ rhs = W.rhs + (size_t)b * P.n_unknowns;
-    const int NUK = P.n_unknowns, CH = P.rhs_chunk;
+    const int NUK = P.n_unknowns, CH = P.rhs_chunk, tf = fresh(tid);
     double *accL = evl;
     int *ptrL = (int *)(accL + ((NUK + 1) & ~1));
     double *gvL = (double *)(ptrL + ((NUK + 4) & ~3)), *wvL = gvL + CH;
-    for (int p = tid; p <= NUK; p += nt) { ptrL[p] = P.rhs_ptr[p]; if (p < NUK) accL[p] = 0.0; }
+    for (int p = tf; p <= NUK; p += nt) { ptrL[p] = P.rhs_ptr[p]; if (p < NUK) accL[p] = 0.0; }
     constexpr int SU = 12;
     for (int c0 = 0; c0 < P.n_rhs_ent; c0 += CH) {
       const int c1 = min(c0 + CH, P.n_rhs_ent);
-      for (int t = c0 + tid; t < c1; t += SU * nt) {
+      for (int t = c0 + tf; t < c1; t += SU * nt) {
         int gp[SU], rw[SU];
 #pragma unroll
         for (int u = 0; u < SU; ++u) { const int tt = min(t + u * nt, c1 - 1); gp[u] = P.rhs_gpos[tt]; rw[u] = P.rhs_row[tt]; }
@@ -1583,7 +1612,7 @@
           if (t + u * nt < c1) { gvL[t + u * nt - c0] = gv[u]; wvL[t + u * nt - c0] = wv[u]; }
       }
       __syncthreads();
-      for (int p = tid; p < NUK; p += nt) {
+      for (int p = tf; p < NUK; p += nt) {
         const int t0 = max(ptrL[p], c0), t1 = min(ptrL[p + 1], c1);
         if (t0 >= t1) continue;
         double acc = accL[p];
diff --git a/quadruped-trajectory-optimization-stack_amd/csrc/model.hpp b/quadruped-trajectory-optimization-stack_amd/csrc/model.hpp
--- a/quadruped-trajectory-optimization-stack_amd/csrc/model.hpp
+++ b/quadruped-trajectory-optimization-stack_amd/csrc/model.hpp
@@ -45,6 +45,7 @@
 };
 constexpr int DYN_LOC = 54;
 constexpr int ROM_LOC = 18;
+constexpr int DYN_VIN = 39, ROM_VIN = 9;
 struct ColDesc {
   int inst, gbase, ncol;
   short kind, dim;
diff --git a/quadruped-trajectory-optimization-stack_amd/csrc/qtos_planner.hip b/quadruped-trajectory-optimization-stack_amd/csrc/qtos_planner.hip
--- a/quadruped-trajectory-optimization-stack_amd/csrc/qtos_planner.hip
+++ b/quadruped-trajectory-optimization-stack_amd/csrc/qtos_planner.hip
@@ -416,54 +416,47 @@
   D.n_force = (int)M.force.size(); D.n_lin = (int)M.linrow.size(); D.n_blocks = (int)M.blocks.size();
   TRY(p->upload(M.dyn, &D.dyn)); TRY(p->upload(M.rom, &D.rom));
   {
-    auto flat = [&](const void *inst0, size_t inst_bytes, size_t n_inst, int n_vec, const i4_t **var, const d2_t **wa, const d2_t **wb) {
+    struct Group { const void *inst0; size_t inst_bytes, n_inst; int n_vec; };
+    auto flat = [&](std::initializer_list<Group> groups, const i4_t **var, const d2_t **wa, const d2_t **wb) {
       std::vector<i4_t> v;
       std::vector<d2_t> a, b;
-      for (size_t i = 0; i < n_inst; ++i)
-        for (int k = 0; k < n_vec; ++k) {
-          const VecIn &in = ((const VecIn *)((const char *)inst0 + i * inst_bytes))[k];
-          for (int d = 0; d < 3; ++d) {
-            v.push_back(i4_t{in.var[d], in.var[3 + d], in.var[6 + d], in.var[9 + d]});
-            a.push_back(d2_t{in.w[0], in.w[1]});
-            b.push_back(d2_t{in.w[2], in.w[3]});
+      for (const Group &G : groups)
+        for (size_t i = 0; i < G.n_inst; ++i)
+          for (int k = 0; k < G.n_vec; ++k) {
+            const VecIn &in = ((const VecIn *)((const char *)G.inst0 + i * G.inst_bytes))[k];
+            for (int d = 0; d < 3; ++d) {
+              v.push_back(i4_t{in.var[d], in.var[3 + d], in.var[6 + d], in.var[9 + d]});
+              a.push_back(d2_t{in.w[0], in.w[1]});
+              b.push_back(d2_t{in.w[2], in.w[3]});
+            }
           }
-        }
       int rc2 = p->upload(v, var);
       if (!rc2) rc2 = p->upload(a, wa);
       if (!rc2) rc2 = p->upload(b, wb);
       return rc2;
     };
     static_assert(DYN_VIN == 39 && ROM_VIN == 9, "13 / 3 input vectors of three components");
-    TRY(flat(M.dyn.data(), sizeof(DynInst), M.dyn.size(), 13, &D.pre_dyn_var, &D.pre_dyn_wa, &D.pre_dyn_wb));
-    TRY(flat(M.rom.data(), sizeof(RomInst), M.rom.size(), 3, &D.pre_rom_var, &D.pre_rom_wa, &D.pre_rom_wb));
+    TRY(flat({{M.dyn.data(), sizeof(DynInst), M.dyn.size(), 13}, {M.rom.data(), sizeof(RomInst), M.rom.size(), 3}}, &D.pre_dyn_var, &D.pre_dyn_wa, &D.pre_dyn_wb));
+    const size_t nd = M.dyn.size() * DYN_VIN;
+    D.pre_rom_var = D.pre_dyn_var + nd; D.pre_rom_wa = D.pre_dyn_wa + nd; D.pre_rom_wb = D.pre_dyn_wb + nd;
   }
   TRY(p->upload(M.force, &D.force)); TRY(p->upload(M.linrow, &D.lin));
+  Symbolic::EvalLayout EL = S.eval_layout(M, 0, env.eval_joint != 0, env.eval_joint != 2);
   {
-    std::map<unsigned long long, int> idx_of;
-    std::vector<double> coefs;
-    bool fits = true;
-    auto ci = [&](double a) {
-      unsigned long long bits;
-      std::memcpy(&bits, &a, 8);
-      auto it = idx_of.find(bits);
-      if (it == idx_of.end()) { it = idx_of.emplace(bits, (int)coefs.size()).first; coefs.push_back(a); }
-      return (unsigned short)it->second;
-    };
-    auto off16 = [&](int off) { if (off < 0 || off > 65535) fits = false; return (unsigned short)off; };
     std::vector<PackedTerm1> d1, r1;
     std::vector<PackedTerm3> d3;
-    for (const LinTerm1 &t : S.dyn_t1) d1.push_back({(unsigned)t.pos, off16(t.off), ci(t.a)});
-    for (const LinTerm1 &t : S.rom_t1) r1.push_back({(unsigned)t.pos, off16(t.off), ci(t.a)});
-    for (const LinTerm3 &t : S.dyn_t3)
-      d3.push_back({(unsigned)t.pos, {off16(t.off[0]), off16(t.off[1]), off16(t.off[2])}, {ci(t.a[0]), ci(t.a[1]), ci(t.a[2])}});
-    if (!fits || coefs.size() > 65535) {
+    std::vector<double> coefs;
+    if (!S.pack_terms(EL.loc_rom - EL.loc_dyn, d1, r1, d3, coefs)) {
       p->err = "Jacobian entry lists exceed the packed format (16-bit offsets / coefficient indices)";
       fprintf(stderr, "qtos: %s\n", p->err.c_str());
       qtos_planner_destroy(p);
       return -4;
     }
     D.n_lin_coef = (int)coefs.size();
-    TRY(p->upload(d1, &D.dyn_t1)); TRY(p->upload(d3, &D.dyn_t3)); TRY(p->upload(r1, &D.rom_t1)); TRY(p->upload(coefs, &D.lin_coef));
+    D.n_dyn_t1 = (int)d1.size(); D.n_dyn_t3 = (int)d3.size();
+    d1.insert(d1.end(), r1.begin(), r1.end());
+    TRY(p->upload(d1, &D.dyn_t1)); TRY(p->upload(d3, &D.dyn_t3)); TRY(p->upload(coefs, &D.lin_coef));
+    D.rom_t1 = D.dyn_t1 + D.n_dyn_t1;
   }
   TRY(p->upload(S.dyn_t1_off, &D.dyn_t1_off)); TRY(p->upload(S.dyn_t3_off, &D.dyn_t3_off));
   D.n_rom_t1 = (int)S.rom_t1.size();
@@ -614,10 +607,12 @@
       if (e != hipSuccess) { p->err = std::string("hipFuncSetAttribute: ") + hipGetErrorString(e); fprintf(stderr, "qtos: %s\n", p->err.c_str()); qtos_planner_destroy(p); return -2; }
     }
   }
-  p->eval_lds = sizeof(double) * (((size_t)M.n_sol + 1) / 2 * 2 + std::max((size_t)DYN_LOC * D.dyn_chunk, (size_t)ROM_LOC * D.rom_chunk) +
-                                  std::max((size_t)DYN_VIN * D.dyn_chunk, (size_t)ROM_VIN * D.rom_chunk));
-  D.coef_in_lds = p->eval_lds + sizeof(double) * (size_t)D.n_lin_coef <= 150 * 1024;
-  if (D.coef_in_lds) p->eval_lds += sizeof(double) * (size_t)D.n_lin_coef;
+  EL = S.eval_layout(M, D.n_lin_coef, EL.joint != 0, env.eval_joint != 2);
+  D.coef_in_lds = EL.coef_in_lds; D.ev_coef_late = EL.coef_late;
+  D.eval_joint = EL.joint;
+  D.ev_loc = EL.loc_dyn; D.ev_loc_rom = EL.loc_rom; D.ev_vin = EL.vin_dyn; D.ev_vin_rom = EL.vin_rom; D.ev_coef = EL.coef;
+  p->eval_lds = EL.bytes();
+  if (env.debug) fprintf(stderr, "qtos: evaluation schedule %s, %zu B of LDS (table %s)\n", EL.joint ? "joint" : "chunked", p->eval_lds, EL.coef_late ? "in LDS over the inputs" : EL.coef_in_lds ? "in LDS" : "in memory");
   {
     D.n_rhs_ent = (int)S.rhs_gpos.size();
     const size_t nuk = (size_t)S.n_unknowns, fixed = ((nuk + 1) & ~(size_t)1) + ((nuk + 4) & ~(size_t)3) / 2;
@@ -625,7 +620,7 @@
     D.rhs_chunk = (int)std::max<size_t>(1, std::min<size_t>(std::min<size_t>((D.n_rhs_ent + ET - 1) / ET, 12), room)) * ET;
     p->eval_lds = std::max(p->eval_lds, (fixed + 2 * (size_t)D.rhs_chunk) * sizeof(double));
   }
-  if (p->eval_lds > 150 * 1024) {
+  if (p->eval_lds > Symbolic::EVAL_LDS_LIMIT) {
     p->err = "too many dynamics knots for the LDS scratch";
     fprintf(stderr, "qtos: evaluation kernels need %zu B of LDS\n", p->eval_lds);
     qtos_planner_destroy(p);
@@ -1315,6 +1310,31 @@
   return (int)d.size();
 }
 
+int qtos_eval_schedule(const QtosPlanner *p) { return p ? p->dp.eval_joint : -1; }
+
+int qtos_analyze_eval_layout(const QtosParams *params, long long *out, int n) {
+  if (!params || !out || n < 0) return -1;
+  const QtosEnv env = QtosEnv::parse();
+  Analysis A;
+  if (analyze_host(*params, env, false, A)) return -1;
+  const auto &[M, S] = A;
+  Symbolic::EvalLayout L = S.eval_layout(M, 0, true);
+  std::vector<PackedTerm1> d1, r1;
+  std::vector<PackedTerm3> d3;
+  std::vector<double> coefs;
+  const bool fits = S.pack_terms(L.joint ? L.loc_rom - L.loc_dyn : 0, d1, r1, d3, coefs);
+  L = S.eval_layout(M, (int)coefs.size(), L.joint != 0, env.eval_joint != 2);
+  long long lo = -1, hi = -1;
+  for (const PackedTerm1 &t : r1) { lo = lo < 0 ? t.off : std::min<long long>(lo, t.off); hi = std::max<long long>(hi, t.off); }
+  const long long v[QTOS_EVAL_LAYOUT_FIELDS] = {
+      L.joint && env.eval_joint, L.joint, (long long)L.bytes(), (long long)Symbolic::EVAL_LDS_LIMIT, L.coef_in_lds + L.coef_late, fits,
+      L.loc_dyn, L.loc_rom, L.vin_dyn, L.vin_rom, L.coef, L.end,
+      (long long)M.dyn.size(), (long long)M.rom.size(), (long long)coefs.size(), (long long)r1.size(), lo, hi};
+  const int k = std::min(n, (int)QTOS_EVAL_LAYOUT_FIELDS);
+  for (int i = 0; i < k; ++i) out[i] = v[i];
+  return k;
+}
+
 int qtos_last_timing_chord(QtosPlanner *p, double *chord_seconds, int *chord_launches) {
   if (!p) return -1;
   if (!p->per_kernel_events) { p->err = "per-kernel events are off (qtos_set_kernel_events)"; return -1; }
diff --git a/quadruped-trajectory-optimization-stack_amd/csrc/symbolic.hpp b/quadruped-trajectory-optimization-stack_amd/csrc/symbolic.hpp
--- a/quadruped-trajectory-optimization-stack_amd/csrc/symbolic.hpp
+++ b/quadruped-trajectory-optimization-stack_amd/csrc/symbolic.hpp
@@ -177,6 +177,59 @@
     }
   }
 
+  bool pack_terms(int rom_base, std::vector<PackedTerm1> &d1, std::vector<PackedTerm1> &r1, std::vector<PackedTerm3> &d3, std::vector<double> &coefs) const {
+    std::map<unsigned long long, int> idx_of;
+    bool fits = true;
+    auto ci = [&](double a) {
+      unsigned long long bits;
+      std::memcpy(&bits, &a, 8);
+      auto it = idx_of.find(bits);
+      if (it == idx_of.end()) { it = idx_of.emplace(bits, (int)coefs.size()).first; coefs.push_back(a); }
+      return (unsigned short)it->second;
+    };
+    auto off16 = [&](int off) { if (off < 0 || off > 65535) fits = false; return (unsigned short)off; };
+    d1.clear(); r1.clear(); d3.clear(); coefs.clear();
+    for (const LinTerm1 &t : dyn_t1) d1.push_back({(unsigned)t.pos, off16(t.off), ci(t.a)});
+    for (const LinTerm1 &t : rom_t1) r1.push_back({(unsigned)t.pos, off16(t.off + rom_base), ci(t.a)});
+    for (const LinTerm3 &t : dyn_t3)
+      d3.push_back({(unsigned)t.pos, {off16(t.off[0]), off16(t.off[1]), off16(t.off[2])}, {ci(t.a[0]), ci(t.a[1]), ci(t.a[2])}});
+    return fits && coefs.size() <= 65535;
+  }
+
+  static constexpr size_t EVAL_LDS_LIMIT = 150 * 1024;
+  struct EvalLayout {
+    int joint = 0, coef_in_lds = 0, coef_late = 0;
+    int loc_dyn = 0, loc_rom = 0, vin_dyn = 0, vin_rom = 0, coef = 0, end = 0;
+    size_t bytes() const { return sizeof(double) * (size_t)end; }
+  };
+  EvalLayout eval_layout(const HostModel &M, int n_lin_coef, bool want_joint, bool late = true) const {
+    const size_t n_dyn = M.dyn.size(), n_rom = M.rom.size(), x = ((size_t)M.n_sol + 1) / 2 * 2;
+    EvalLayout L;
+    const size_t side = x + (size_t)(DYN_LOC + DYN_VIN) * n_dyn + (size_t)(ROM_LOC + ROM_VIN) * n_rom;
+    L.joint = want_joint && (size_t)M.dyn_chunk >= n_dyn && (size_t)rom_chunk >= n_rom && sizeof(double) * side <= EVAL_LDS_LIMIT;
+    L.loc_dyn = (int)x;
+    int vin_end;
+    if (L.joint) {
+      L.loc_rom = L.loc_dyn + DYN_LOC * (int)n_dyn;
+      L.vin_dyn = L.loc_rom + ROM_LOC * (int)n_rom;
+      L.vin_rom = L.vin_dyn + DYN_VIN * (int)n_dyn;
+      vin_end = L.vin_rom + ROM_VIN * (int)n_rom;
+    } else {
+      L.loc_rom = L.loc_dyn;
+      L.vin_dyn = L.vin_rom = L.loc_dyn + std::max(DYN_LOC * M.dyn_chunk, ROM_LOC * rom_chunk);
+      vin_end = L.vin_dyn + std::max(DYN_VIN * M.dyn_chunk, ROM_VIN * rom_chunk);
+    }
+    L.coef = L.end = vin_end;
+    if (sizeof(double) * ((size_t)vin_end + (size_t)n_lin_coef) <= EVAL_LDS_LIMIT) {
+      L.coef_in_lds = 1;
+      L.end = vin_end + n_lin_coef;
+    } else if (L.joint && late && L.vin_dyn + n_lin_coef <= vin_end) {
+      L.coef_in_lds = L.coef_late = 1;
+      L.coef = L.vin_dyn;
+    }
+    return L;
+  }
+
   static constexpr int SHDR_INTS = 8;
   int REC_MAX_DOUBLES = 2048, REC_MAX_INTS = 6144;
   int rec_cap_ints = 0;
```

New measurement: 110,700 (median of 6 runs). No clear change (+0.9%).
